# OATML-Markslab/ProteinGym

Hardware: AMD Instinct MI355X
Metric: mutants scored/sec (ESM-1v 650M masked-marginal) (higher is better)
Workload: dtype f16x3 (fp32 operands split into 2 fp16 planes, 3 fp16 MFMAs per product, fp32 accumulate)

## Files before the change

### proteingym_amd/csrc/api_esm.hip

```cpp
#include "model.h"

namespace pgmi {

int create_esm(pgmi_model* m, const pgmi_config* cfg, const float* w, int64_t n_weights) {
    BlobCursor c(m, w, n_weights);
    walk_esm(c);
    return c.finish();
}

void walk_esm_layer(BlobCursor& c, Layer* Lp, size_t F) {
    pgmi_model* m = c.m;
    const size_t D = m->cfg.embed_dim, dh = m->dh, Da = m->Da;
    auto slot = [&](size_t col) -> size_t { return rotate_half_slot(col, dh); };
    const float qscale = 1.0f / sqrtf((float)dh);
    std::vector<float> wq(3 * Da * D, 0.0f), bq(3 * Da, 0.0f), wo_r(D * Da, 0.0f);
    Layer& L = *Lp;
    c.upload(&L.ln1_w, D);
    c.upload(&L.ln1_b, D);
    pack_qkv_slots(c.take(3 * (D * D + D)), D, Da, slot, qscale, wq.data(), bq.data());
    c.linear(&L.wqkv, &L.wqkv16, wq.data(), wq.size(), D);
    c.upload(&L.bqkv, bq.data(), bq.size());
    pack_out_cols(c.take(D * D), D, Da, slot, wo_r.data());
    c.linear(&L.wo, &L.wo16, wo_r.data(), wo_r.size(), Da);
    c.upload(&L.bo, D);
    c.upload(&L.ln2_w, D);
    c.upload(&L.ln2_b, D);
    c.linear(&L.w1, &L.w116, F * D, D);
    c.upload(&L.b1, F);
    c.linear(&L.w2, &L.w216, D * F, F);
    c.upload(&L.b2, D);
}

void walk_esm(BlobCursor& c) {
    pgmi_model* m = c.m;
    const pgmi_config* cfg = &m->cfg;
    const size_t D = cfg->embed_dim, V = cfg->vocab;
    c.upload(&m->embed_tokens, V * D);
    if (cfg->arch == PGMI_ARCH_ESM1B) c.upload(&m->embed_positions, (size_t)(cfg->max_positions + 2) * D);
    if (cfg->emb_layer_norm_before) {
        c.upload(&m->lnb_w, D);
        c.upload(&m->lnb_b, D);
    }
    m->layers.resize(cfg->layers);
    for (int l = 0; l < cfg->layers; ++l) walk_esm_layer(c, &m->layers[l], cfg->ffn_dim);
    c.upload(&m->lna_w, D);
    c.upload(&m->lna_b, D);
    c.linear(&m->hd_w, &m->hd16, D * D, D);
    c.upload(&m->hd_b, D);
    c.upload(&m->hln_w, D);
    c.upload(&m->hln_b, D);
    c.upload(&m->head_b, V);
    m->head_w = m->embed_tokens;
}

int ensure_rotary(pgmi_model* m, int T) {
    if ((!esm2_rotary(m->cfg.arch) && !esmc_blocks(m->cfg.arch)) || T <= m->rot_len) return PGMI_OK;
    return upload_rotate_half(m, std::max(T, 1026));
}

int upload_rotate_half(pgmi_model* m, int n) {
    const int rh = m->rot_halves;
    float inv[64];
    const int half = m->dh / 2;
    for (int i = 0; i < half; ++i) inv[i] = 1.0f / powf(10000.0f, (float)(2 * i) / (float)m->dh);
    return upload_rotary(m, n, rh, [&](int t, int g, int i) {
        const int j = (rh == 1) ? i : 32 * g + i;
        return j < half ? (float)t * inv[j] : 0.0f;
    });
}

int encoder_layer(pgmi_model* m, const Layer& L, int B, int T, bool rotary, const int32_t* keep, int n_keep, bool* compacted) {
    const pgmi_config& c = m->cfg;
    const int M = B * T, D = c.embed_dim, F = L.ffn ? L.ffn : c.ffn_dim, N1 = L.ffn ? L.ffn : m->fc1_cols, H = c.heads, Da = m->Da;
    hipStream_t s = m->stream;
    int rc = PGMI_OK;
    const double ln_bytes = 2.0 * M * D * 4;
    const int prec = c.precision;
    const int mode16 = (prec == PGMI_PREC_F16X3) ? 1 : 2;
    { ProfScope p(m, PGMI_K_LAYERNORM, 0, ln_bytes);
      if (prec == PGMI_PREC_FP32) launch_layernorm(m->x, L.ln1_w, L.ln1_b, M, D, 1e-5f, m->h, s);
      else launch_layernorm16(m->x, L.ln1_w, L.ln1_b, M, D, 1e-5f, m->h16, mode16, s); }
    const bool fused_qkv = prec != PGMI_PREC_FP32 && !L.q_ln;
    { ProfScope p(m, PGMI_K_GEMM_QKV, 2.0 * M * 3 * D * D, 0);
      if (fused_qkv) {
          GemmLaunch g = qkv_launch(m, L.wqkv16, L.bqkv, M, Da, D, T, m->Hs);
          g.bf = prec == PGMI_PREC_BF16;
          g.qkv.cos_t = m->rot_cos; g.qkv.sin_t = m->rot_sin; g.qkv.rotary = rotary; g.qkv.rot_halves = m->rot_halves;
          rc = launch_gemm16(g);
      } else
          rc = linear(m, m->h, m->h16, L.wqkv, L.wqkv16, L.bqkv, nullptr, m->qkv, nullptr, M, 3 * Da, D, EPI_NONE);
      if (rc) return rc; }
    { ProfScope p(m, PGMI_K_ATTENTION, 4.0 * M * T * D, L.q_ln ? (double)M * D * 20 : 0);
      if (L.q_ln && (rc = launch_qkln_prep(m->qkv, L.q_ln, L.k_ln, 1e-5f, m->rot_cos, m->rot_sin, B, T, H, m->qk16, m->qk16_plane,
                                           m->vt16, m->vt16_plane, s)))
          return rc;
      const bool v2 = prec != PGMI_PREC_FP32;
      if (rotary && !v2) launch_rotary(m->qkv, m->rot_cos, m->rot_sin, M, T, m->Hs, s, m->rot_halves);
      if (v2) {
          AttLaunch a;
          a.qk16 = m->qk16, a.qk_plane = m->qk16_plane, a.vt16 = m->vt16, a.vt_plane = m->vt16_plane;
          a.B = B, a.T = T, a.H = H, a.head_dim = m->rot_halves * kHeadDim;
          a.kv_len = m->kv_len;
          a.out = prec == PGMI_PREC_F16X3 ? ATT_OUT_SPLIT : ATT_OUT_BF16;
          a.ctx16 = m->h16;
          a.stream = s;
          rc = launch_attention_f16x3_v2(a);
      } else {
          rc = launch_attention_f32(m->qkv, m->kv_len, B, T, H, m->h, s, m->rot_halves * kHeadDim);
      }
      if (rc) return rc; }
    if (keep && !L.g_norm_w) {
        const int R = n_keep;
        ProfScope p(m, PGMI_K_KEPT_ROWS, 2.0 * R * D * (Da + N1 + F), 0);
        launch_gather_rows(m->x, keep, R, D, m->qkv, s);
        if (prec == PGMI_PREC_FP32) launch_gather_rows(m->h, keep, R, Da, m->g, s);
        else
            launch_gather_rows(reinterpret_cast<const float*>(m->h16), keep, R, prec == PGMI_PREC_F16X3 ? Da : Da / 2,
                               reinterpret_cast<float*>(m->g16), s);
        rc = linear(m, m->g, m->g16, L.wo, L.wo16, L.bo, m->qkv, m->x, nullptr, R, D, Da, EPI_NONE);
        if (rc) return rc;
        if (prec == PGMI_PREC_FP32) launch_layernorm(m->x, L.ln2_w, L.ln2_b, R, D, 1e-5f, m->h, s);
        else launch_layernorm16(m->x, L.ln2_w, L.ln2_b, R, D, 1e-5f, m->h16, mode16, s);
        rc = linear(m, m->h, m->h16, L.w1, L.w116, L.b1, nullptr,
                    prec == PGMI_PREC_FP32 ? m->g : nullptr, prec == PGMI_PREC_FP32 ? nullptr : m->g16,
                    R, N1, D, m->fc1_epi);
        if (rc) return rc;
        rc = linear(m, m->g, m->g16, L.w2, L.w216, L.b2, m->x, m->x, nullptr, R, D, F, EPI_NONE);
        if (rc) return rc;
        if (compacted) *compacted = true;
        return PGMI_OK;
    }
    { ProfScope p(m, PGMI_K_GEMM_OUT, 2.0 * M * D * D, 0);
      rc = linear(m, m->h, m->h16, L.wo, L.wo16, L.bo, m->x, m->x, nullptr, M, D, Da, EPI_NONE);
      if (rc) return rc; }
    if (L.g_norm_w && m->e3_framed && (rc = geom_branch(m, L, B, T))) return rc;
    { ProfScope p(m, PGMI_K_LAYERNORM, 0, ln_bytes);
      if (prec == PGMI_PREC_FP32) launch_layernorm(m->x, L.ln2_w, L.ln2_b, M, D, 1e-5f, m->h, s);
      else launch_layernorm16(m->x, L.ln2_w, L.ln2_b, M, D, 1e-5f, m->h16, mode16, s); }
    { ProfScope p(m, PGMI_K_GEMM_FC1, 2.0 * M * N1 * D, 0);
      rc = linear(m, m->h, m->h16, L.w1, L.w116, L.b1, nullptr,
                  prec == PGMI_PREC_FP32 ? m->g : nullptr, prec == PGMI_PREC_FP32 ? nullptr : m->g16,
                  M, N1, D, m->fc1_epi);
      if (rc) return rc; }
    { ProfScope p(m, PGMI_K_GEMM_FC2, 2.0 * M * F * D, 0);
      rc = linear(m, m->g, m->g16, L.w2, L.w216, L.b2, m->x, m->x, nullptr, M, D, F, EPI_NONE);
      if (rc) return rc; }
    return PGMI_OK;
}

int run_encoder(pgmi_model* m, int B, int T, const int32_t* keep, int n_keep, bool* compacted) {
    const pgmi_config& c = m->cfg;
    const int M = B * T, D = c.embed_dim;
    hipStream_t s = m->stream;
    if (c.arch == PGMI_ARCH_ESM1B && T > c.max_positions) {
        set_error("Sequence length %d above maximum sequence length of %d", T, c.max_positions);
        return PGMI_EINVAL;
    }
    int rc = ensure_rotary(m, T);
    if (!rc) rc = reset_pad_keys(m, B, T);
    if (rc) return rc;
    {
        ProfScope p(m, PGMI_K_EMBED, 0, (double)M * D * 4);
        launch_seq_stats(m->tokens, B, T, m->embed_gather ? 0 : c.token_dropout, m->denom, m->pos_idx, m->kv_len, s, m->mask_id);
        if (c.arch == PGMI_ARCH_ESM3) { if ((rc = esm3_embed(m, B, T))) return rc; }
        else if (c.arch == PGMI_ARCH_MULAN) { if ((rc = mulan_embed(m, B, T))) return rc; }
        else if (m->embed_gather) launch_gather_rows(m->embed_tokens, m->tokens, M, D, m->x, s);
        else launch_embed(m->tokens, m->denom, m->pos_idx, m->embed_tokens, m->embed_positions, c.token_dropout, M, T, D, m->x, s, m->mask_id);
        if (m->lnb_w) {
            launch_layernorm(m->x, m->lnb_w, m->lnb_b, M, D, 1e-5f, m->x, s);
            launch_zero_pad_rows(m->tokens, M, D, m->x, s);
        }
    }
    for (int l = 0; l < c.layers; ++l) {
        const bool kept = keep && m->keep_rows && l == c.layers - 1;
        if ((rc = encoder_layer(m, m->layers[l], B, T, esm2_rotary(c.arch), kept ? keep : nullptr, n_keep, compacted))) return rc;
    }
    PGMI_HIP(hipGetLastError());
    return PGMI_OK;
}

int run_head(pgmi_model* m, int R, const int32_t* row_idx) {
    const pgmi_config& c = m->cfg;
    ProfScope p(m, PGMI_K_HEAD, 2.0 * R * c.embed_dim * (c.embed_dim + c.vocab), 0);
    int rc = head_hidden(m, R, row_idx);
    if (rc) return rc;
    launch_vocab_logsoftmax(m->g, m->head_w, m->head_b, R, c.embed_dim, c.vocab, m->lp, m->nonfinite, m->stream);
    PGMI_HIP(hipGetLastError());
    return PGMI_OK;
}

int head_hidden(pgmi_model* m, int R, const int32_t* row_idx) {
    const pgmi_config& c = m->cfg;
    const int D = c.embed_dim;
    hipStream_t s = m->stream;
    const int prec = c.precision;
    const float* src = m->x;
    if (row_idx) {
        launch_gather_rows(m->x, row_idx, R, D, m->h, s);
        src = m->h;
    }
    if (prec == PGMI_PREC_FP32) launch_layernorm(src, m->lna_w, m->lna_b, R, D, 1e-5f, m->h, s);
    else launch_layernorm16(src, m->lna_w, m->lna_b, R, D, 1e-5f, m->h16, prec == PGMI_PREC_F16X3 ? 1 : 2, s);
    int rc = linear(m, m->h, m->h16, m->hd_w, m->hd16, m->hd_b, nullptr, m->g, nullptr, R, D, D, EPI_GELU);
    if (rc) return rc;
    launch_layernorm(m->g, m->hln_w, m->hln_b, R, D, 1e-5f, m->g, s);
    return PGMI_OK;
}


int run_rows(pgmi_model* m, int B, int T, int R, const int32_t* row_idx) {
    bool compacted = false;
    int rc = run_encoder(m, B, T, row_idx, R, &compacted);
    if (rc) return rc;
    return run_head(m, R, compacted ? nullptr : row_idx);
}

}

extern "C" {

int pgmi_token_logprobs(pgmi_model* m, const int32_t* tokens, int B, int T, float* out) {
    if (!m || !tokens || !out || B <= 0 || T <= 0) { set_error("bad argument"); return PGMI_EINVAL; }
    if (m->cfg.arch == PGMI_ARCH_SAPROT) { set_error("SaProt models are scored with pgmi_saprot_token_logprobs / pgmi_saprot_group_logprobs"); return PGMI_EINVAL; }
    if (m->cfg.arch == PGMI_ARCH_MULAN) { set_error("MULAN models are scored with pgmi_mulan_token_logprobs / pgmi_mulan_set_logprobs"); return PGMI_EINVAL; }
    if (T + 31 > m->max_rows) { set_error("T=%d exceeds workspace rows %d", T, m->max_rows); return PGMI_EINVAL; }
    int rc = check_tokens(tokens, B, T);
    if (rc) return rc;
    PGMI_HIP(hipSetDevice(m->device));
    const int V = m->cfg.vocab;
    rc = for_each_chunk(m, B, T, [&](int b0, int bc) {
        PGMI_HIP(hipMemcpyAsync(m->tokens, tokens + (size_t)b0 * T, (size_t)bc * T * 4, hipMemcpyHostToDevice, m->stream));
        int rc = run_rows(m, bc, T, bc * T, nullptr);
        if (rc) return rc;
        PGMI_HIP(hipMemcpyAsync(out + (size_t)b0 * T * V, m->lp, (size_t)bc * T * V * 4, hipMemcpyDeviceToHost, m->stream));
        return PGMI_OK;
    });
    return rc ? rc : check_nonfinite(m);
}

int pgmi_masked_logprobs(pgmi_model* m, const int32_t* tokens, const int32_t* mask_pos, int B, int T, float* out) {
    if (!m || !tokens || !mask_pos || !out || B <= 0 || T <= 0) { set_error("bad argument"); return PGMI_EINVAL; }
    if (m->cfg.arch == PGMI_ARCH_SAPROT) { set_error("SaProt models are scored with pgmi_saprot_token_logprobs / pgmi_saprot_group_logprobs"); return PGMI_EINVAL; }
    if (m->cfg.arch == PGMI_ARCH_MULAN) { set_error("MULAN models are scored with pgmi_mulan_token_logprobs / pgmi_mulan_set_logprobs"); return PGMI_EINVAL; }
    if (esmc_blocks(m->cfg.arch) && T + 31 > m->max_rows) { set_error("T=%d exceeds workspace rows %d", T, m->max_rows); return PGMI_EINVAL; }
    if (T > m->max_rows) { set_error("T=%d exceeds workspace rows %d", T, m->max_rows); return PGMI_EINVAL; }
    int rc = check_tokens(tokens, B, T);
    if (rc) return rc;
    for (int b = 0; b < B; ++b)
        if (mask_pos[b] < 0 || mask_pos[b] >= T) { set_error("mask_pos[%d]=%d out of range", b, mask_pos[b]); return PGMI_EINVAL; }
    PGMI_HIP(hipSetDevice(m->device));
    const int V = m->cfg.vocab;
    std::vector<int32_t> ridx;
    rc = for_each_chunk(m, B, T, [&](int b0, int bc) {
        ridx.resize(bc);
        for (int b = 0; b < bc; ++b) ridx[b] = b * T + mask_pos[b0 + b];
        PGMI_HIP(hipMemcpyAsync(m->tokens, tokens + (size_t)b0 * T, (size_t)bc * T * 4, hipMemcpyHostToDevice, m->stream));
        PGMI_HIP(hipMemcpyAsync(m->aux_i, mask_pos + b0, (size_t)bc * 4, hipMemcpyHostToDevice, m->stream));
        PGMI_HIP(hipMemcpyAsync(m->row_idx, ridx.data(), (size_t)bc * 4, hipMemcpyHostToDevice, m->stream));
        launch_apply_mask(m->tokens, m->aux_i, bc, T, m->stream);
        int rc = run_rows(m, bc, T, bc, m->row_idx);
        if (rc) return rc;
        PGMI_HIP(hipMemcpyAsync(out + (size_t)b0 * V, m->lp, (size_t)bc * V * 4, hipMemcpyDeviceToHost, m->stream));
        return PGMI_OK;
    });
    return rc ? rc : check_nonfinite(m);
}

int pgmi_assay_create(pgmi_model* m, const int32_t* wt_tokens, int n_tok, const int32_t* positions, int P,
                      int window, const int32_t* sub_pos, const int32_t* sub_wt, const int32_t* sub_mt,
                      const int64_t* mut_off, int64_t n_mut, pgmi_assay** out) {
    if (!out) { set_error("null out"); return PGMI_EINVAL; }
    *out = nullptr;
    if (!m || !wt_tokens || n_tok <= 0 || P < 0 || (P > 0 && !positions) || window <= 0 || n_mut < 0) { set_error("bad argument"); return PGMI_EINVAL; }
    if (esmc_blocks(m->cfg.arch)) { set_error("ESM C / ESM3 assays run through pgmi_masked_logprobs (their window rule is not pgmi_optimal_window)"); return PGMI_EINVAL; }
    if (m->cfg.arch == PGMI_ARCH_SAPROT) { set_error("SaProt assays run through pgmi_saprot_group_logprobs (position sets, no window)"); return PGMI_EINVAL; }
    if (m->cfg.arch == PGMI_ARCH_MULAN) { set_error("MULAN assays run through pgmi_mulan_set_logprobs (position sets, no window)"); return PGMI_EINVAL; }
    for (int i = 0; i < n_tok; ++i)
        if (wt_tokens[i] < 0 || wt_tokens[i] >= PGMI_VOCAB || wt_tokens[i] == PGMI_TOK_PAD) { set_error("wt token %d invalid at %d", wt_tokens[i], i); return PGMI_EINVAL; }
    const int T = std::min(n_tok, window);
    if (T > m->max_rows) { set_error("T=%d exceeds workspace rows %d", T, m->max_rows); return PGMI_EINVAL; }
    std::vector<int32_t> ws(P), mr(P);
    for (int i = 0; i < P; ++i) {
        if (positions[i] < 0 || positions[i] >= n_tok) { set_error("position %d out of range", positions[i]); return PGMI_EINVAL; }
        int s, e;
        pgmi_optimal_window(positions[i], n_tok, window, &s, &e);
        if (e - s != T) { set_error("internal: window length %d != %d", e - s, T); return PGMI_EINVAL; }
        ws[i] = s;
        mr[i] = positions[i] - s;
    }
    const int64_t n_sub = n_mut ? mut_off[n_mut] : 0;
    for (int64_t k = 0; k < n_sub; ++k)
        if (sub_pos[k] < 0 || sub_pos[k] >= n_tok || sub_wt[k] < 0 || sub_wt[k] >= PGMI_VOCAB || sub_mt[k] < 0 || sub_mt[k] >= PGMI_VOCAB) {
            set_error("substitution %lld out of range", (long long)k);
            return PGMI_EINVAL;
        }
    PGMI_HIP(hipSetDevice(m->device));
    pgmi_assay* a = new pgmi_assay();
    a->m = m; a->n_tok = n_tok; a->P = P; a->T = T; a->n_mut = n_mut; a->n_sub = n_sub;
    int rc = dev_upload(a->allocs, &a->wt, wt_tokens, (size_t)n_tok);
    if (!rc) rc = dev_upload(a->allocs, &a->positions, positions, (size_t)P);
    if (!rc) rc = dev_upload(a->allocs, &a->win_start, ws.data(), (size_t)P);
    if (!rc) rc = dev_upload(a->allocs, &a->mask_rel, mr.data(), (size_t)P);
    if (!rc) rc = dev_upload(a->allocs, &a->sub_pos, sub_pos, (size_t)n_sub);
    if (!rc) rc = dev_upload(a->allocs, &a->sub_wt, sub_wt, (size_t)n_sub);
    if (!rc) rc = dev_upload(a->allocs, &a->sub_mt, sub_mt, (size_t)n_sub);
    if (!rc) rc = dev_upload(a->allocs, &a->mut_off, mut_off, (size_t)(n_mut + 1));
    if (!rc) rc = dev_alloc(a->allocs, &a->table, (size_t)n_tok * PGMI_VOCAB);
    if (!rc) rc = dev_alloc(a->allocs, &a->scores, (size_t)n_mut);
    if (rc) { pgmi_assay_destroy(a); return rc; }
    m->assays.push_back(a);
    *out = a;
    return PGMI_OK;
}

void pgmi_assay_destroy(pgmi_assay* a) {
    if (!a) return;
    if (a->m) {
        hipSetDevice(a->m->device);
        hipStreamSynchronize(a->m->stream);
        auto& v = a->m->assays;
        v.erase(std::remove(v.begin(), v.end(), a), v.end());
    }
    for (void* p : a->allocs) hipFree(p);
    delete a;
}

int pgmi_assay_run(pgmi_model* m, pgmi_assay* a, double* scores_host, float* table_host, double* scores_dev) {
    if (!m || !a || a->m != m) { set_error("bad model/assay handle (assay belongs to another or a destroyed model)"); return PGMI_EINVAL; }
    PGMI_HIP(hipSetDevice(m->device));
    hipStream_t s = m->stream;
    const int T = a->T, V = m->cfg.vocab;
    const int per = rows_per_chunk(m, T);
    launch_fill_f32(a->table, (int64_t)a->n_tok * V, NAN, s);
    for (int p0 = 0; p0 < a->P; p0 += per) {
        const int bc = std::min(per, a->P - p0);
        launch_make_masked_windows(a->wt, a->win_start + p0, a->mask_rel + p0, bc, T, m->tokens, s);
        launch_row_index(a->mask_rel + p0, bc, T, m->row_idx, s);
        int rc = run_rows(m, bc, T, bc, m->row_idx);
        if (rc) return rc;
        launch_scatter_rows(m->lp, a->positions + p0, bc, V, a->table, s);
    }
    {
        ProfScope p(m, PGMI_K_SCORE, 0, (double)a->n_sub * 20);
        launch_score_mutants(a->table, V, a->sub_pos, a->sub_wt, a->sub_mt, a->mut_off, a->n_mut, a->scores, s);
    }
    PGMI_HIP(hipGetLastError());
    if (scores_dev && a->n_mut) PGMI_HIP(hipMemcpyAsync(scores_dev, a->scores, (size_t)a->n_mut * 8, hipMemcpyDeviceToDevice, s));
    if (scores_host && a->n_mut) PGMI_HIP(hipMemcpyAsync(scores_host, a->scores, (size_t)a->n_mut * 8, hipMemcpyDeviceToHost, s));
    if (table_host) PGMI_HIP(hipMemcpyAsync(table_host, a->table, (size_t)a->n_tok * V * 4, hipMemcpyDeviceToHost, s));
    PGMI_HIP(hipStreamSynchronize(s));
    return check_nonfinite(m);
}

int pgmi_pppl_create(pgmi_model* m, const uint8_t* tokens, const int64_t* seq_off, int64_t n_seq, pgmi_pppl** out) {
    if (!out) { set_error("null out"); return PGMI_EINVAL; }
    *out = nullptr;
    if (!m || !tokens || !seq_off || n_seq <= 0 || n_seq > 0x7fffffff) { set_error("bad argument"); return PGMI_EINVAL; }
    if (m->cfg.arch != PGMI_ARCH_ESM1B && m->cfg.arch != PGMI_ARCH_ESM2) { set_error("pseudo-ppl needs an ESM-1b/1v/ESM2 model"); return PGMI_EINVAL; }
    if (seq_off[0] != 0) { set_error("seq_off[0] must be 0"); return PGMI_EINVAL; }
    for (int64_t n = 0; n < n_seq; ++n) {
        const int64_t len = seq_off[n + 1] - seq_off[n];
        if (len < 2 || len > (1 << 24)) { set_error("sequence %lld has %lld tokens", (long long)n, (long long)len); return PGMI_EINVAL; }
        const uint8_t* t = tokens + seq_off[n];
        for (int64_t i = 0; i < len; ++i)
            if (t[i] >= PGMI_VOCAB || t[i] == PGMI_TOK_PAD) { set_error("token id %d invalid at sequence %lld, position %lld", (int)t[i], (long long)n, (long long)i); return PGMI_EINVAL; }
    }
    PGMI_HIP(hipSetDevice(m->device));
    pgmi_pppl* q = new pgmi_pppl();
    q->m = m;
    q->N = n_seq;
    q->off.assign(seq_off, seq_off + n_seq + 1);
    int rc = dev_upload(q->allocs, &q->tok8, tokens, (size_t)seq_off[n_seq]);
    if (!rc) rc = dev_upload(q->allocs, &q->off_dev, seq_off, (size_t)n_seq + 1);
    if (rc) { for (void* p : q->allocs) hipFree(p); delete q; return rc; }
    m->pppls.push_back(q);
    *out = q;
    return PGMI_OK;
}

void pgmi_pppl_destroy(pgmi_pppl* q) {
    if (!q) return;
    if (q->m) {
        hipSetDevice(q->m->device);
        hipStreamSynchronize(q->m->stream);
        auto& v = q->m->pppls;
        v.erase(std::remove(v.begin(), v.end(), q), v.end());
    }
    for (void* p : q->allocs) hipFree(p);
    delete q;
}

int64_t pgmi_pppl_rows(const pgmi_pppl* q, int64_t first, int64_t count) {
    if (!q || first < 0 || count < 0 || first + count > q->N) return -1;
    int64_t r = 0;
    for (int64_t n = first; n < first + count; ++n) r += std::max<int64_t>(0, q->off[n + 1] - q->off[n] - 4);
    return r;
}

int pgmi_pppl_run(pgmi_model* m, pgmi_pppl* q, int64_t first, int64_t count, double* scores_host, float* terms_host,
                  double* scores_dev) {
    if (!m || !q || q->m != m) { set_error("bad model/library handle (library belongs to another or a destroyed model)"); return PGMI_EINVAL; }
    if (first < 0 || count <= 0 || first + count > q->N) { set_error("sequence range [%lld, %lld) outside the library of %lld", (long long)first, (long long)(first + count), (long long)q->N); return PGMI_EINVAL; }
    PGMI_HIP(hipSetDevice(m->device));
    hipStream_t s = m->stream;
    const int J = (int)count, V = m->cfg.vocab;
    std::vector<int32_t> sid(J);
    for (int j = 0; j < J; ++j) sid[j] = (int32_t)(first + j);
    auto len_of = [&](int32_t n) { return q->off[n + 1] - q->off[n]; };
    std::stable_sort(sid.begin(), sid.end(), [&](int32_t a, int32_t b) { return len_of(a) > len_of(b); });
    std::vector<int64_t> rp((size_t)J + 1);
    rp[0] = 0;
    for (int j = 0; j < J; ++j) rp[j + 1] = rp[j] + std::max<int64_t>(0, len_of(sid[j]) - 4);
    const int64_t R = rp[J];
    const int64_t Tmax = len_of(sid[0]);
    if (R > 0 && Tmax + 31 > m->max_rows) { set_error("T=%lld exceeds workspace rows %d", (long long)Tmax, m->max_rows); return PGMI_EINVAL; }
    if (R > 0 && m->cfg.arch == PGMI_ARCH_ESM1B && Tmax > m->cfg.max_positions) {
        set_error("Sequence length %lld above maximum sequence length of %d", (long long)Tmax, m->cfg.max_positions);
        return PGMI_EINVAL;
    }
    std::vector<void*> pool;
    auto cleanup = [&]() { for (void* p : pool) hipFree(p); };
    int32_t* d_sid = nullptr;
    int64_t* d_rp = nullptr;
    float* d_terms = nullptr;
    double* d_out = nullptr;
    int rc = dev_upload(pool, &d_sid, sid.data(), (size_t)J);
    if (!rc) rc = dev_upload(pool, &d_rp, rp.data(), (size_t)J + 1);
    if (!rc) rc = dev_alloc(pool, &d_terms, (size_t)R);
    if (!rc) rc = dev_alloc(pool, &d_out, (size_t)J);
    if (rc) { cleanup(); return rc; }
    q->last_rows = R; q->last_chunks = 0; q->last_tokens = 0; q->last_padded = 0;
    int j0 = 0;
    for (int64_t g0 = 0; g0 < R;) {
        while (rp[j0 + 1] <= g0) ++j0;
        const int T = (int)len_of(sid[j0]);
        const int bc = (int)std::min<int64_t>(rows_per_chunk(m, T), R - g0);
        launch_make_pppl_rows(q->tok8, q->off_dev, d_sid, d_rp, J, g0, bc, T, m->tokens, m->row_idx, m->aux_i, s);
        rc = run_rows(m, bc, T, bc, m->row_idx);
        if (rc) { hipStreamSynchronize(s); cleanup(); return rc; }
        launch_pppl_pick(m->lp, m->aux_i, bc, V, d_terms + g0, s);
        q->last_chunks += 1;
        q->last_padded += (int64_t)bc * T;
        g0 += bc;
        if ((q->last_chunks & 63) == 0 && g0 < R && (rc = check_nonfinite(m)) != PGMI_OK) { cleanup(); return rc; }
    }
    for (int j = 0; j < J; ++j) q->last_tokens += (rp[j + 1] - rp[j]) * len_of(sid[j]);
    {
        ProfScope p(m, PGMI_K_SCORE, 0, (double)R * 4);
        launch_pppl_sum(d_terms, d_rp, d_sid, J, first, d_out, s);
    }
    hipError_t e = hipGetLastError();
    if (e == hipSuccess && scores_dev) e = hipMemcpyAsync(scores_dev, d_out, (size_t)J * 8, hipMemcpyDeviceToDevice, s);
    if (e == hipSuccess && scores_host) e = hipMemcpyAsync(scores_host, d_out, (size_t)J * 8, hipMemcpyDeviceToHost, s);
    std::vector<float> sorted_terms;
    if (e == hipSuccess && terms_host && R > 0) {
        sorted_terms.resize((size_t)R);
        e = hipMemcpyAsync(sorted_terms.data(), d_terms, (size_t)R * 4, hipMemcpyDeviceToHost, s);
    }
    if (e == hipSuccess) e = hipStreamSynchronize(s);
    cleanup();
    if (e != hipSuccess) { set_error("pseudo-ppl run failed: %s", hipGetErrorString(e)); return PGMI_EHIP; }
    if (terms_host && R > 0) {
        std::vector<int64_t> dst((size_t)J + 1, 0);
        for (int k = 0; k < J; ++k) dst[k + 1] = dst[k] + std::max<int64_t>(0, len_of((int32_t)(first + k)) - 4);
        for (int j = 0; j < J; ++j)
            std::copy(sorted_terms.begin() + rp[j], sorted_terms.begin() + rp[j + 1], terms_host + dst[sid[j] - first]);
    }
    return check_nonfinite(m);
}

int pgmi_pppl_stats(const pgmi_pppl* q, int64_t* rows, int64_t* chunks, int64_t* tokens, int64_t* padded_tokens) {
    if (!q) { set_error("null library"); return PGMI_EINVAL; }
    if (rows) *rows = q->last_rows;
    if (chunks) *chunks = q->last_chunks;
    if (tokens) *tokens = q->last_tokens;
    if (padded_tokens) *padded_tokens = q->last_padded;
    return PGMI_OK;
}

}
```

### proteingym_amd/csrc/api_model.hip

```cpp
#include "model.h"

namespace pgmi {

static thread_local char g_err[1024] = "";
void set_error(const char* fmt, ...) {
    va_list ap;
    va_start(ap, fmt);
    vsnprintf(g_err, sizeof(g_err), fmt, ap);
    va_end(ap);
}

int prof_drain(pgmi_model* m) {
    if (m->events_used == 0) return PGMI_OK;
    PGMI_HIP(hipStreamSynchronize(m->stream));
    for (size_t i = 0; i < m->events_used; ++i) {
        float ms = 0.f;
        PGMI_HIP(hipEventElapsedTime(&ms, m->events[i].start, m->events[i].stop));
        m->prof_ms[m->events[i].cls] += ms;
    }
    m->events_used = 0;
    return PGMI_OK;
}

int check_cfg(const pgmi_config* c) {
// ... 240 lines not shown
    if (c->emb_layer_norm_before) n += 2 * D;
    n += (int64_t)c->layers * (2 * D + 4 * (D * D + D) + 2 * D + (F * D + F) + (D * F + D));
    n += 2 * D + (D * D + D) + 2 * D + V;
    return n;
}

int pgmi_model_create(const pgmi_config* cfg, const float* w, int64_t n_weights, int device, pgmi_model** out) {
    if (cfg && cfg->arch == PGMI_ARCH_PROGEN2) {
        if (out) *out = nullptr;
        set_error("ProGen2 models are created with pgmi_pg2_model_create (it takes rotary_dim)");
        return PGMI_EINVAL;
    }
    if (cfg && cfg->arch == PGMI_ARCH_GPT) {
        if (out) *out = nullptr;
        set_error("causal decoder models are created with pgmi_gpt_model_create (it takes pos_kind)");
        return PGMI_EINVAL;
    }
    if (cfg && cfg->arch == PGMI_ARCH_SAPROT) {
        if (out) *out = nullptr;
        set_error("SaProt models are created with pgmi_saprot_model_create (it takes the tokenizer's <mask> id)");
        return PGMI_EINVAL;
    }
    if (cfg && cfg->arch == PGMI_ARCH_MULAN) {
        if (out) *out = nullptr;
        set_error("MULAN models are created with pgmi_mulan_model_create (it takes the <mask> id and the vocabulary's groups)");
        return PGMI_EINVAL;
    }
    if (cfg && cfg->arch == PGMI_ARCH_POET) {
        if (out) *out = nullptr;
        set_error("PoET models are created with pgmi_poet_model_create (it takes final_norm)");
        return PGMI_EINVAL;
    }
    if (cfg && cfg->arch == PGMI_ARCH_PROGEN3) {
        if (out) *out = nullptr;
        set_error("ProGen3 models are created with pgmi_pg3_model_create (it takes pgmi_pg3_params)");
        return PGMI_EINVAL;
    }
    if (cfg && cfg->arch == PGMI_ARCH_ESM3) {
        if (out) *out = nullptr;
        set_error("ESM3 models are created with pgmi_esm3_model_create (it takes v_heads)");
        return PGMI_EINVAL;
    }
    if (cfg && cfg->arch == PGMI_ARCH_ESMIF1) {
        if (out) *out = nullptr;
        set_error("ESM-IF1 decoders are created with pgmi_esmif1_model_create (it takes the encoder width)");
        return PGMI_EINVAL;
    }
    return model_create(cfg, w, n_weights, device, out, 0);
}

}

namespace pgmi {

static int alloc_workspace(pgmi_model* m) {
    const pgmi_config& c = m->cfg;
    const size_t R = m->max_rows, D = c.embed_dim, V = c.vocab, Da = m->Da;
    const size_t F = c.arch == PGMI_ARCH_MULAN ? std::max<size_t>(c.ffn_dim, 4 * D) : c.ffn_dim;
    const size_t Dw = std::max(D, Da);
    const bool f32mode = c.precision == PGMI_PREC_FP32;
    int rc = PGMI_OK;
    auto alloc = [&](auto** p, size_t n) { if (!rc) rc = dev_alloc(m->allocs, p, n); };
    alloc(&m->x, R * D);
    alloc(&m->h, R * Dw);
    alloc(&m->qkv, R * 3 * Da);
    alloc(&m->g, R * (f32mode ? std::max(F, D) : D));
    if (!f32mode) {
        const size_t planes = c.precision == PGMI_PREC_F16X3 ? 2 : 1;
        m->h16_plane = R * Dw;
        m->g16_plane = R * F;
        alloc(&m->h16, m->h16_plane * planes);
        alloc(&m->g16, m->g16_plane * planes);
    }
    alloc(&m->nonfinite, (size_t)1);
    if (!f32mode) {
        m->qk16_plane = R * 2 * Da;
        m->vt16_plane = R * Da;
        alloc(&m->qk16, m->qk16_plane * 2);
        alloc(&m->vt16, m->vt16_plane * 2);
    }
    if (c.arch == PGMI_ARCH_MSA) {
        alloc(&m->xt, R * D);
        alloc(&m->msa_kv_len, (size_t)2048);
    }
    alloc(&m->lp, ((c.arch == PGMI_ARCH_GPT || c.arch == PGMI_ARCH_PROGEN3) && V > kWave ? (size_t)m->gpt_head_rows : R) * V);
    alloc(&m->denom, R);
    alloc(&m->tokens, R);
    alloc(&m->pos_idx, R);
    alloc(&m->kv_len, R);
    alloc(&m->row_idx, R);
    alloc(&m->aux_i, R);
    if (rc) return rc;
    PGMI_HIP(hipMemset(m->nonfinite, 0, 4));
    if (m->vt16) PGMI_HIP(hipMemset(m->vt16, 0, m->vt16_plane * 2 * sizeof(unsigned short)));
    return PGMI_OK;
}

int model_create(const pgmi_config* cfg, const float* w, int64_t n_weights, int device, pgmi_model** out, int arch_arg,
                 const pgmi_pg3_params* pg3) {
    if (!out) { set_error("null out"); return PGMI_EINVAL; }
    *out = nullptr;
    int rc = check_cfg(cfg);
    if (rc) return rc;
    if (cfg->arch == PGMI_ARCH_PROGEN3 && (rc = pg3_check(cfg, pg3))) return rc;
    if (cfg->arch == PGMI_ARCH_ESM3 && (rc = esm3_check(cfg, arch_arg))) return rc;
    if (cfg->arch == PGMI_ARCH_ESMIF1 && (rc = if1_check(cfg, arch_arg))) return rc;
    const int64_t need = cfg->arch == PGMI_ARCH_GPT ? gpt_weight_count(cfg, arch_arg)
                         : cfg->arch == PGMI_ARCH_PROGEN3 ? pg3_weight_count(cfg, pg3)
                         : cfg->arch == PGMI_ARCH_POET ? poet_weight_count(cfg, arch_arg)
                         : cfg->arch == PGMI_ARCH_ESM3 ? esm3_weight_count(cfg, arch_arg)
                         : cfg->arch == PGMI_ARCH_ESMIF1 ? if1_weight_count(cfg, arch_arg)
                         : cfg->arch == PGMI_ARCH_MULAN ? mulan_weight_count(cfg) : pgmi_weight_count(cfg);
    if (need < 0) { set_error("causal decoder pos_kind %d: must be PGMI_GPT_POS_ROTARY or PGMI_GPT_POS_LEARNED", arch_arg); return PGMI_EINVAL; }
    if (!w || n_weights != need) {
        set_error("weight blob has %lld elements, config needs %lld", (long long)n_weights, (long long)need);
        return PGMI_EINVAL;
    }
    const int ndev = pgmi_device_count();
    if (ndev <= 0) { set_error("no HIP device visible (libpgmi has no CPU fallback)"); return PGMI_ENODEV; }
    if (device < 0 || device >= ndev) { set_error("device %d out of range (%d visible)", device, ndev); return PGMI_EINVAL; }
    PGMI_HIP(hipSetDevice(device));
    pgmi_model* m = new pgmi_model();
    m->cfg = *cfg;
    m->device = device;
    if (hipStreamCreateWithFlags(&m->stream, hipStreamNonBlocking) != hipSuccess) { set_error("hipStreamCreate failed"); delete m; return PGMI_EHIP; }
    m->dh = cfg->embed_dim / cfg->heads;
    m->rot_halves = m->dh > 2 * kHeadDim ? 4 : m->dh > kHeadDim ? 2 : 1;
    m->Hs = cfg->heads * m->rot_halves;
    m->Da = m->Hs * kHeadDim;
    m->ln_eps = cfg->ln_eps > 0.f ? cfg->ln_eps : 1e-5f;
    m->max_rows = std::max(cfg->max_rows > 0 ? cfg->max_rows : 98304, 2048);
    const size_t V = cfg->vocab;
    const std::vector<float> zeros(std::max({3 * (size_t)m->Da, (V + 63) / 64 * 64, (size_t)cfg->embed_dim, V, (size_t)cfg->heads}), 0.0f);
    rc = dev_upload(m->allocs, &m->zeros, zeros.data(), zeros.size());
    m->fc1_cols = cfg->ffn_dim;
    if (!rc) switch (cfg->arch) {
        case PGMI_ARCH_TRANCEPTION: rc = create_tranception(m, cfg, w, n_weights); break;
        case PGMI_ARCH_MSA: rc = create_msa(m, cfg, w, n_weights); break;
        case PGMI_ARCH_PROGEN2: rc = create_progen2(m, cfg, w, n_weights, arch_arg); break;
        case PGMI_ARCH_GPT: rc = create_gpt(m, cfg, w, n_weights, arch_arg); break;
        case PGMI_ARCH_ESMC: rc = create_esmc(m, cfg, w, n_weights); break;
        case PGMI_ARCH_SAPROT: rc = create_saprot(m, cfg, w, n_weights, arch_arg); break;
        case PGMI_ARCH_MULAN: rc = create_mulan(m, cfg, w, n_weights, arch_arg); break;
        case PGMI_ARCH_POET: rc = create_poet(m, cfg, w, n_weights, arch_arg); break;
        case PGMI_ARCH_PROGEN3: rc = create_progen3(m, cfg, w, n_weights, pg3); break;
        case PGMI_ARCH_ESM3: rc = create_esm3(m, cfg, w, n_weights, arch_arg); break;
        case PGMI_ARCH_ESMIF1: rc = create_esmif1(m, cfg, w, n_weights, arch_arg); break;
        default: rc = create_esm(m, cfg, w, n_weights);
    }
    if (!rc) rc = alloc_workspace(m);
    if (rc) { pgmi_model_destroy(m); return rc; }
    m->keep_rows = env_int("PGMI_KEEP_ROWS", 1);
    gemm_options_from_env();
    m->gemm_variant = env_int("PGMI_GEMM_VARIANT", 0);
    *out = m;
    return PGMI_OK;
}

}

namespace pgmi {

int side_open(pgmi_model* pm, const char* name, const float* w, int64_t n_weights, int64_t want, bool scan_finite, int device, int precision,
              hipStream_t lend) {
    if (!w || n_weights != want) {
        set_error("%s weight blob has %lld elements, config needs %lld", name, (long long)n_weights, (long long)want);
        return PGMI_EINVAL;
    }
    for (int64_t i = 0; scan_finite && i < n_weights; ++i)
        if (!std::isfinite(w[i])) { set_error("%s: weight blob element %lld is not finite", name, (long long)i); return PGMI_EINVAL; }
    int n_dev = 0;
    if (hipGetDeviceCount(&n_dev) != hipSuccess || n_dev <= 0) { set_error("no HIP device (libpgmi has no CPU fallback)"); return PGMI_ENODEV; }
    if (device < 0 || device >= n_dev) { set_error("device %d out of range (%d visible)", device, n_dev); return PGMI_EINVAL; }
    PGMI_HIP(hipSetDevice(device));
    gemm_options_from_env();
    pm->device = device;
    pm->cfg.precision = precision;
    if (lend) pm->stream = lend;
    else if (hipStreamCreate(&pm->stream) != hipSuccess) { set_error("hipStreamCreate failed"); return PGMI_EHIP; }
    return PGMI_OK;
}

int side_sync(pgmi_model* pm, int rc, const char* what) {
    const hipError_t e1 = hipGetLastError(), e2 = hipStreamSynchronize(pm->stream);
    if (!rc && (e1 != hipSuccess || e2 != hipSuccess)) {
        set_error("%s failed: %s", what, hipGetErrorString(e1 != hipSuccess ? e1 : e2));
        rc = PGMI_EHIP;
    }
    return rc;
}

int overflow_error(int precision) {
    set_error("non-finite log-probabilities%s", precision == PGMI_PREC_F16X3
              ? ": an activation left the fp16 range in precision f16x3; re-run with precision fp32" : "");
    return PGMI_EOVERFLOW;
}

void side_release(pgmi_model* pm, bool own_stream) {
    hipSetDevice(pm->device);
    if (pm->stream) hipStreamSynchronize(pm->stream);
    for (ProfEvent& e : pm->events) { hipEventDestroy(e.start); hipEventDestroy(e.stop); }
    for (void* p : pm->allocs) hipFree(p);
    if (pm->stream && own_stream) hipStreamDestroy(pm->stream);
}

}

extern "C" {

void pgmi_model_destroy(pgmi_model* m) {
    if (!m) return;
    hipSetDevice(m->device);
    if (m->stream) hipStreamSynchronize(m->stream);
    for (pgmi_assay* a : m->assays) {
        for (void* p : a->allocs) hipFree(p);
        a->allocs.clear();
        a->m = nullptr;
    }
    m->assays.clear();
    for (pgmi_pppl* q : m->pppls) {
        for (void* p : q->allocs) hipFree(p);
        q->allocs.clear();
        q->m = nullptr;
    }
    m->pppls.clear();
    for (auto& e : m->events) { hipEventDestroy(e.start); hipEventDestroy(e.stop); }
    if (m->moe.counts_host) hipHostFree(m->moe.counts_host);
    for (void* p : m->allocs) hipFree(p);
    if (m->stream) hipStreamDestroy(m->stream);
    delete m;
}

int pgmi_model_device(const pgmi_model* m) { return m ? m->device : -1; }

int pgmi_set_option(const char* name, int64_t value) {
    if (!name) { set_error("null option name"); return PGMI_EINVAL; }
    int rc = gemm_set_option(name, (long long)value);
    if (rc) rc = att_set_option(name, (long long)value);
    if (rc) rc = eve_set_option(name, (long long)value);
    if (rc) rc = mpnn_set_option(name, (long long)value);
    if (rc) rc = unirep_set_option(name, (long long)value);
    if (rc) rc = s2f_set_option(name, (long long)value);
    if (rc) set_error("unknown option '%s' (gemm_half_tail, gemm_max_rows, att_xcd_local, att_v3, eve_max_rows, eve_fixed_sample, eve_prior_batch, mpnn_max_rows, unirep_max_rows, s2f_max_rows)", name);
    return rc;
}

int pgmi_synchronize(pgmi_model* m) {
    if (!m) { set_error("null model"); return PGMI_EINVAL; }
    PGMI_HIP(hipStreamSynchronize(m->stream));
    return PGMI_OK;
}

int pgmi_profile_enable(pgmi_model* m, int on) {
    if (!m) { set_error("null model"); return PGMI_EINVAL; }
    int rc = prof_drain(m);
    m->prof = on != 0;
    return rc;
}

int pgmi_profile_reset(pgmi_model* m) {
    if (!m) { set_error("null model"); return PGMI_EINVAL; }
    int rc = prof_drain(m);
    for (int i = 0; i < PGMI_K_COUNT; ++i) { m->prof_ms[i] = 0; m->prof_n[i] = 0; m->prof_flops[i] = 0; m->prof_bytes[i] = 0; }
    return rc;
}

int pgmi_profile_get(pgmi_model* m, int k, double* ms, int64_t* launches, double* flops, double* bytes) {
    if (!m || k < 0 || k >= PGMI_K_COUNT) { set_error("bad argument"); return PGMI_EINVAL; }
    int rc = prof_drain(m);
    if (rc) return rc;
    if (ms) *ms = m->prof_ms[k];
    if (launches) *launches = m->prof_n[k];
    if (flops) *flops = m->prof_flops[k];
    if (bytes) *bytes = m->prof_bytes[k];
    return PGMI_OK;
}

}
```

### proteingym_amd/csrc/attention_f16.hip

```cpp
#include <stdlib.h>
#include <string.h>
#include <algorithm>

#include "attention_f16_common.h"

namespace pgmi {

template <int WPB, int OUT, int NSTG, int DH = 64, bool RAG = false, int DO = DH>
__global__ __launch_bounds__(WPB * 64) void attention_f16x3_v2_kernel(
    const unsigned short* __restrict__ qk16, size_t qk_plane, const unsigned short* __restrict__ vt16,
    size_t vt_plane, const int32_t* __restrict__ kv_len, const float* __restrict__ slopes, int T, int H,
    int Tp, float* __restrict__ ctx, unsigned short* __restrict__ ctx16, RagMap rag, int dense_nblk, int nseq) {
    constexpr float defer_thr = kAttDefer;
    constexpr int NT = WPB * 64;
    constexpr int KCPR = DH / 8;
    constexpr int KCH = AKT * KCPR, VCH = DO * 4;
    constexpr int NSL = DH / DO;
    static_assert(NSL == 1 || (OUT == ATT_OUT_SPLIT && !RAG), "sliced context: split-plane output of dense launches only");
    constexpr int STG_CH = 2 * KCH + 2 * VCH;
    constexpr int NWI = STG_CH / 64;
    static_assert(NWI % WPB == 0, "the wave-instructions of a stage divide evenly over the waves");
    constexpr int NDMA = NWI / WPB;
    constexpr int NS = DH / 16, ND = DO / 32;
    extern __shared__ __attribute__((aligned(16))) u32x4 lds[];
// ... 108 lines not shown
            for (int s = 0; s < NS; ++s) {
                const int ci = r * KCPR + ((2 * s + kh) ^ k_swizzle<DH>(r));
                qh[s] = qbase[ci];
                ql[s] = qbase[KCH + ci];
            }
        }
        asm volatile("s_waitcnt lgkmcnt(0)" ::: "memory");
        __builtin_amdgcn_s_barrier();
        asm volatile("" ::: "memory");
#pragma unroll
        for (int t = 1; t < NSTG - 1; ++t)
            if (t < nkt) issue_tile(t, t);
    } else {
#pragma unroll
        for (int t = 0; t < NSTG - 1; ++t)
            if (t < nkt) issue_tile(t, t);
    }

    f32x16 om[ND], oc[ND];
#pragma unroll
    for (int dt = 0; dt < ND; ++dt)
#pragma unroll
        for (int v = 0; v < 16; ++v) { om[dt][v] = 0.f; oc[dt][v] = 0.f; }
    float m_run = -INFINITY, l_run = 0.f;
    constexpr float kInvLo = 1.0f / kLoScale;

    const f32x16 zero16 = {0.f, 0.f, 0.f, 0.f, 0.f, 0.f, 0.f, 0.f, 0.f, 0.f, 0.f, 0.f, 0.f, 0.f, 0.f, 0.f};
    auto wanted = [&](int kt) -> bool { return active && !(causal && kt * AKT > q0 + 31); };
    auto scores = [&](int buf, f32x16& sm, f32x16& sc) {
        const u32x4* Kb = lds + buf * STG_CH;
#pragma unroll
        for (int s = 0; s < NS; ++s) {
            const int ci = r * KCPR + ((2 * s + kh) ^ k_swizzle<DH>(r));
            const u32x4 kfh = Kb[ci], kfl = Kb[KCH + ci];
            sc = mfma_h(kfh, ql[s], s == 0 ? zero16 : sc);
            sc = mfma_h(kfl, qh[s], sc);
            sm = mfma_h(kfh, qh[s], s == 0 ? zero16 : sm);
        }
    };
    auto wait_tile = [&](int younger) {
        if (younger >= 2) asm volatile("s_waitcnt vmcnt(%0)" ::"n"(2 * NDMA) : "memory");
        else if (younger == 1) asm volatile("s_waitcnt vmcnt(%0)" ::"n"(NDMA) : "memory");
        else asm volatile("s_waitcnt vmcnt(0)" ::: "memory");
    };
    int cur = 0;
    for (int kt = 0; kt < nkt; ++kt) {
        wait_tile(min(NSTG - 2, nkt - 1 - kt));
        __builtin_amdgcn_s_barrier();
        asm volatile("" ::: "memory");
        if (kt + NSTG - 1 < nkt) issue_tile(kt + NSTG - 1, (cur == 0) ? NSTG - 1 : cur - 1);
        if (wanted(kt)) {
            const u32x4* Vb = lds + cur * STG_CH + 2 * KCH;
            f32x16 sm, sc;
            scores(cur, sm, sc);
            float st[16];
            if (causal) {
                const float kb = (float)(kt * AKT + 4 * kh);
#pragma unroll
                for (int v = 0; v < 16; ++v)
                    st[v] = fmaf(slope2, kb + (float)((v & 3) + 8 * (v >> 2)), fmaf(sc[v], kInvLo, sm[v]));
                if (kt * AKT + AKT - 1 > q0) {
#pragma unroll
                    for (int v = 0; v < 16; ++v) {
                        const int key = kt * AKT + (v & 3) + 8 * (v >> 2) + 4 * kh;
                        if (key > q0 + r) st[v] = -INFINITY;
                    }
                }
            } else {
#pragma unroll
                for (int v = 0; v < 16; ++v) st[v] = fmaf(sc[v], kInvLo, sm[v]);
            }
            if (kt * AKT + AKT > Tk) {
#pragma unroll
                for (int v = 0; v < 16; ++v) {
                    const int key = kt * AKT + (v & 3) + 8 * (v >> 2) + 4 * kh;
                    if (key >= Tk) st[v] = -INFINITY;
                }
            }
            float mloc = st[0];
#pragma unroll
            for (int v = 1; v < 16; ++v) mloc = fmaxf(mloc, st[v]);
            {
                const unsigned int mu = __builtin_bit_cast(unsigned int, mloc);
                const auto sw = __builtin_amdgcn_permlane32_swap(mu, mu, false, false);
                const unsigned int s0 = sw[0], s1 = sw[1];
                mloc = fmaxf(__builtin_bit_cast(float, s0), __builtin_bit_cast(float, s1));
            }
            const float m_new = fmaxf(m_run, mloc);
            if (!__all(m_new <= m_run + defer_thr)) {
                const bool moved = m_new > m_run + defer_thr;
                const float alpha = moved ? __builtin_amdgcn_exp2f(m_run - m_new) : 1.0f;
                l_run *= alpha;
#pragma unroll
                for (int dt = 0; dt < ND; ++dt)
#pragma unroll
                    for (int v = 0; v < 16; ++v) { om[dt][v] *= alpha; oc[dt][v] *= alpha; }
                if (moved) m_run = m_new;
            }
            const float mb = m_run - 10.0f;
            typedef float f32x2 __attribute__((ext_vector_type(2)));
#pragma unroll
            for (int v = 0; v < 16; v += 2) {
                const f32x2 dlt = f32x2{st[v], st[v + 1]} - f32x2{mb, mb};
                st[v] = __builtin_amdgcn_exp2f(dlt[0]);
                st[v + 1] = __builtin_amdgcn_exp2f(dlt[1]);
            }
            l_run += ((st[0] + st[1]) + (st[2] + st[3])) + ((st[4] + st[5]) + (st[6] + st[7])) +
                     (((st[8] + st[9]) + (st[10] + st[11])) + ((st[12] + st[13]) + (st[14] + st[15])));
#pragma unroll
            for (int m = 0; m < 2; ++m) {
                u32x4 ph, pl;
#pragma unroll
                for (int e = 0; e < 4; ++e) {
                    const u32x2 p = split_p(st[8 * m + 2 * e], st[8 * m + 2 * e + 1]);
                    ph[e] = p[0];
                    pl[e] = p[1];
                }
#pragma unroll
                for (int dt = 0; dt < ND; ++dt) {
                    const int ci = v_chunk(dt * 32 + r, m, kh);
                    const u32x4 vfh = Vb[ci], vfl = Vb[VCH + ci];
                    oc[dt] = mfma_h(vfh, pl, oc[dt]);
                    oc[dt] = mfma_h(vfl, ph, oc[dt]);
                    om[dt] = mfma_h(vfh, ph, om[dt]);
                }
            }
        }
        cur = (cur == NSTG - 1) ? 0 : cur + 1;
    }

    if (active) {
        const float l_tot = l_run + __shfl_xor(l_run, 32);
        const float inv = 1.0f / l_tot;
        const bool row_ok = q0 + r < T && q0 + r >= p0;
        const size_t orow = (size_t)(orow0 + max(min(q0 + r, T - 1), p0));
        if (OUT == ATT_OUT_BF16) store_ctx_bf16<ND>(om, oc, inv, kInvLo, row_ok, ctx16 + orow * (size_t)D + (size_t)h * DH, kh);
        else if (OUT == ATT_OUT_SPLIT) store_ctx_split<ND>(om, oc, inv, kInvLo, row_ok, ctx16 + orow * (size_t)(2 * D) + (size_t)((h * DH + d0) / 32) * 64, kh);
        else if (row_ok) store_ctx_f32<ND>(om, oc, inv, kInvLo, ctx + (size_t)(orow0 + q0 + r) * D + (size_t)h * DH + 4 * kh);
    }
}


using Att16v2Kernel = decltype(&attention_f16x3_v2_kernel<4, ATT_OUT_F32, 3, 64, false, 64>);
struct Att16v2Inst { int wpb, out, head_dim; bool rag; Att16v2Kernel fn; size_t lds_bytes; };
template <int WPB, int OUT, int NSTG, int DH, bool RAG = false, int DO = DH>
static constexpr Att16v2Inst att16v2_inst() {
    return {WPB, OUT, DH, RAG, attention_f16x3_v2_kernel<WPB, OUT, NSTG, DH, RAG, DO>, (size_t)NSTG * (8 * DH + 8 * DO) * 16};
}
static const Att16v2Inst kAtt16v2[] = {
    att16v2_inst<1, ATT_OUT_F32, 3, 64>(),   att16v2_inst<2, ATT_OUT_F32, 3, 64>(),   att16v2_inst<4, ATT_OUT_F32, 3, 64>(),
    att16v2_inst<1, ATT_OUT_SPLIT, 3, 64>(), att16v2_inst<2, ATT_OUT_SPLIT, 3, 64>(), att16v2_inst<4, ATT_OUT_SPLIT, 3, 64>(),
    att16v2_inst<1, ATT_OUT_BF16, 3, 64>(),  att16v2_inst<2, ATT_OUT_BF16, 3, 64>(),  att16v2_inst<4, ATT_OUT_BF16, 3, 64>(),
    att16v2_inst<1, ATT_OUT_SPLIT, 3, 64, true>(), att16v2_inst<2, ATT_OUT_SPLIT, 3, 64, true>(), att16v2_inst<4, ATT_OUT_SPLIT, 3, 64, true>(),
    att16v2_inst<4, ATT_OUT_F32, 3, 128>(),  att16v2_inst<4, ATT_OUT_SPLIT, 3, 128>(), att16v2_inst<4, ATT_OUT_BF16, 3, 128>(),
    att16v2_inst<4, ATT_OUT_SPLIT, 2, 256, false, 128>(),
};

static int launch_att16v2(const AttLaunch& a, int wpb, dim3 grid, const RagMap* rag, int dense_nblk) {
    for (const Att16v2Inst& k : kAtt16v2) {
        if (k.wpb != wpb || k.out != a.out || k.head_dim != a.head_dim || k.rag != (rag != nullptr)) continue;
        if (k.lds_bytes > 65536) {
            hipError_t e = hipFuncSetAttribute(reinterpret_cast<const void*>(k.fn), hipFuncAttributeMaxDynamicSharedMemorySize, (int)k.lds_bytes);
            if (e != hipSuccess) { set_error("hipFuncSetAttribute: %s", hipGetErrorString(e)); return PGMI_EHIP; }
        }
        hipLaunchKernelGGL(k.fn, grid, dim3(wpb * 64), k.lds_bytes, a.stream, a.qk16, a.qk_plane, a.vt16, a.vt_plane, a.kv_len, a.slopes,
                           a.T, a.H, (a.T + 31) / 32 * 32, a.ctx, a.ctx16, rag ? *rag : RagMap{}, dense_nblk, a.B);
        PGMI_HIP(hipGetLastError());
        return PGMI_OK;
    }
    set_error("attention_f16x3_v2: no kernel for %d waves, output %d, head_dim %d%s", wpb, (int)a.out, a.head_dim, rag ? ", ragged" : "");
    return PGMI_EINVAL;
}

static int g_att_xcd_local = -1;
int att_set_option(const char* name, long long value) {
    if (!strcmp(name, "att_xcd_local")) { g_att_xcd_local = (int)value; return PGMI_OK; }
    if (!strcmp(name, "att_v3")) { att_v3_set_option((int)value); return PGMI_OK; }
    return PGMI_EINVAL;
}
static dim3 dense_grid(int nblk, int H, int B, int* dense_nblk) {
    if (g_att_xcd_local == 0 || (g_att_xcd_local < 0 && nblk < 2)) { *dense_nblk = 0; return dim3(nblk, H, B); }
    *dense_nblk = nblk;
    const long long pairs = (long long)H * B, groups = (pairs + 7) / 8;
    return dim3((unsigned)(groups * 8 * nblk), 1, 1);
}

int att16_waves_per_block(int T) {
    const int n32 = (T + 31) / 32, nblk = (n32 + 3) / 4;
    const int wpb = (n32 + nblk - 1) / nblk;
    return wpb == 3 ? 4 : wpb;
}

static int check_operand_range(const char* who, const AttLaunch& a) {
    const unsigned long long Tp = (unsigned long long)(a.T + 31) / 32 * 32;
    const unsigned long long seq_bytes = (unsigned long long)a.T * 2ull * (unsigned long long)a.H * (unsigned long long)a.head_dim * 2ull;
    const unsigned long long vt_bytes = (unsigned long long)a.head_dim * Tp * 2ull;
    if ((unsigned long long)a.qk_plane * 2ull + seq_bytes >= (1ull << 32) || (unsigned long long)a.vt_plane * 2ull + vt_bytes >= (1ull << 32)) {
        set_error("%s: operand planes of %zu / %zu halfs exceed the 32-bit offset range of the K / V^T DMA "
                  "(plane stride + one sequence must stay below 4 GiB: create the model with a smaller max_rows)", who, a.qk_plane, a.vt_plane);
        return PGMI_EINVAL;
    }
    return PGMI_OK;
}

int launch_attention_f16x3_v2(const AttLaunch& a) {
    const int B = a.B, T = a.T, H = a.H, head_dim = a.head_dim;
    if (B <= 0 || T <= 0 || H <= 0 || a.out < ATT_OUT_F32 || a.out > ATT_OUT_BF16 || (head_dim != 64 && head_dim != 128 && head_dim != 256)) {
        set_error("attention_f16x3_v2: bad arguments B=%d T=%d H=%d out=%d head_dim=%d", B, T, H, (int)a.out, head_dim);
        return PGMI_EINVAL;
    }
    const int n32 = (T + 31) / 32, Tp = n32 * 32;
    int rc = check_operand_range("attention_f16x3_v2", a);
    if (rc) return rc;
    int dn = 0;
    if (head_dim == 256) {
        if (a.qkv || a.conv || !a.slopes || a.out != ATT_OUT_SPLIT) { set_error("attention_f16x3_v2: head_dim 256 is the causal, fused-QKV, split-plane-output flavour only"); return PGMI_EINVAL; }
        const dim3 grid = dense_grid((n32 + 3) / 4, 2 * H, B, &dn);
        return launch_att16v2(a, 4, grid, nullptr, dn);
    }
    if (head_dim == 128) {
        if (a.qkv || a.conv) { set_error("attention_f16x3_v2: head_dim 128 needs operands from the fused QKV projection"); return PGMI_EINVAL; }
        const dim3 grid = dense_grid((n32 + 3) / 4, H, B, &dn);
        return launch_att16v2(a, 4, grid, nullptr, dn);
    }
    if (a.qkv && a.conv && a.rotary) { set_error("attention_f16x3_v2: depth-wise convolution and rotary together are not a model this library knows"); return PGMI_EINVAL; }
    if (a.qkv && a.conv && H % 4) { set_error("attention_f16x3_v2: the depth-wise convolution has four head groups, H = %d is not a multiple of 4", H); return PGMI_EINVAL; }
    if (a.qkv && a.conv)
        launch_qkv_prep_conv(dim3(n32, H, B), a.stream, a.qkv, a.conv, T, H, Tp, a.qk16, a.qk_plane, a.vt16, a.vt_plane, nullptr);
    else if (a.qkv)
        launch_qkv_prep(dim3(n32, H, B), a.stream, a.qkv, a.cos_t, a.sin_t, a.rotary, T, H, Tp, a.qk16, a.qk_plane, a.vt16, a.vt_plane);
    const int wpb = att16_waves_per_block(T);
    const dim3 grid = dense_grid((n32 + wpb - 1) / wpb, H, B, &dn);
    return att_v3_serves(a) ? launch_att16v3(a, wpb, grid, dn) : launch_att16v2(a, wpb, grid, nullptr, dn);
}

int launch_attention_tr_ragged(const AttLaunch& a, const AttRagged& rg) {
    const int T = a.T, H = a.H;
    if (T <= 0 || H <= 0 || !a.qkv || !a.conv || !a.slopes || a.head_dim != 64 || a.out != ATT_OUT_SPLIT || rg.n_tiles <= 0 || rg.n_blocks <= 0) {
        set_error("attention_tr_ragged: bad arguments T=%d H=%d tiles=%d blocks=%d", T, H, rg.n_tiles, rg.n_blocks);
        return PGMI_EINVAL;
    }
    const int rc = check_operand_range("attention_tr_ragged", a);
    if (rc) return rc;
    const RagMap tiles{rg.seq_off, rg.seq_p, rg.seq_q, rg.seq_root, rg.seq_vt, rg.tile_seq, rg.tile_j};
    launch_qkv_prep_conv(dim3(rg.n_tiles, H, 1), a.stream, a.qkv, a.conv, T, H, (T + 31) / 32 * 32, a.qk16, a.qk_plane, a.vt16, a.vt_plane, &tiles);
    const RagMap rag{rg.seq_off, rg.seq_p, rg.seq_q, rg.seq_root, rg.seq_vt, rg.blk_seq, rg.blk_j};
    return launch_att16v2(a, att16_waves_per_block(T), dim3(rg.n_blocks, H, 1), &rag, 0);
}

}
```

### proteingym_amd/csrc/common.h

```cpp
#pragma once
#include <hip/hip_runtime.h>
#include <stdint.h>
#include <stddef.h>

#include "../../include/pgmi.h"

namespace pgmi {

void set_error(const char* fmt, ...);

#define PGMI_HIP(expr)                                                                   \
    do {                                                                                 \
        hipError_t _e = (expr);                                                          \
        if (_e != hipSuccess) {                                                          \
            pgmi::set_error("%s failed: %s (%s:%d)", #expr, hipGetErrorString(_e),       \
                            __FILE__, __LINE__);                                         \
            return PGMI_EHIP;                                                            \
        }                                                                                \
    } while (0)

typedef float f32x4 __attribute__((ext_vector_type(4)));
typedef float f32x16 __attribute__((ext_vector_type(16)));

constexpr int kWave = 64;
constexpr int kHeadDim = 64;

enum Epilogue { EPI_NONE = 0, EPI_GELU = 1, EPI_SQRELU = 2, EPI_GELU_TANH = 3,
                EPI_SWIGLU = 4,
                EPI_RELU = 5 };

constexpr float kLoScale = 2048.0f;
constexpr float kQLog2e = 1.4426950408889634f;

__host__ __device__ __forceinline__ size_t ki_off(size_t row, int k, int K) {
    return row * (size_t)(2 * K) + (size_t)(k >> 5) * 64 + (size_t)(k & 31);
}
#if defined(__HIPCC__)
__device__ __forceinline__ void split_act(float x, _Float16& hi, _Float16& lo) {
    hi = (fabsf(x) < 6.103515625e-05f) ? (_Float16)0.0f : (_Float16)x;
    lo = (_Float16)((x - (float)hi) * kLoScale);
}
typedef _Float16 f16x4 __attribute__((ext_vector_type(4)));
__device__ __forceinline__ void split_act4(f32x4 x, f16x4& hi, f16x4& lo) {
    f32x4 xz, lo32;
#pragma unroll
    for (int e = 0; e < 4; ++e) xz[e] = (fabsf(x[e]) < 6.103515625e-05f) ? 0.0f : x[e];
    hi = __builtin_convertvector(xz, f16x4);
    const f32x4 xs = x * f32x4{kLoScale, kLoScale, kLoScale, kLoScale};
#pragma unroll
    for (int e = 0; e < 4; ++e) lo32[e] = __builtin_fmaf((float)hi[e], -kLoScale, xs[e]);
    lo = __builtin_convertvector(lo32, f16x4);
}
__device__ __forceinline__ void split_act4_prod(f32x4 a, f32x4 b, f16x4& hi, f16x4& lo) {
    const f32x4 x = a * b;
    f32x4 xz, lo32;
#pragma unroll
    for (int e = 0; e < 4; ++e) xz[e] = (fabsf(x[e]) < 6.103515625e-05f) ? 0.0f : x[e];
    hi = __builtin_convertvector(xz, f16x4);
#pragma unroll
    for (int e = 0; e < 4; ++e) lo32[e] = __builtin_fmaf(a[e], b[e], -(float)hi[e]);
    lo = __builtin_convertvector(lo32 * f32x4{kLoScale, kLoScale, kLoScale, kLoScale}, f16x4);
}
__device__ __forceinline__ void store_split4(f32x4 o, unsigned short* y16, size_t row, int c, int lane, int D) {
    typedef _Float16 h4 __attribute__((ext_vector_type(4)));
    typedef unsigned int u32x2 __attribute__((ext_vector_type(2)));
    typedef unsigned int u32x4 __attribute__((ext_vector_type(4)));
    h4 hi, lo;
#pragma unroll
    for (int k = 0; k < 4; ++k) {
        _Float16 a, b;
        split_act(o[k], a, b);
        hi[k] = a;
        lo[k] = b;
    }
    const u32x2 H = __builtin_bit_cast(u32x2, hi), L = __builtin_bit_cast(u32x2, lo);
    const bool odd = lane & 1;
    const unsigned int s0 = odd ? H[0] : L[0], s1 = odd ? H[1] : L[1];
    const unsigned int r0 = __shfl_xor(s0, 1), r1 = __shfl_xor(s1, 1);
    const u32x4 out = odd ? u32x4{r0, r1, L[0], L[1]} : u32x4{H[0], H[1], r0, r1};
    *reinterpret_cast<u32x4*>(y16 + ki_off(row, 4 * (c & ~1), D) + (odd ? 32 : 0)) = out;
}
#endif

void launch_make_masked_windows(const int32_t* wt, const int32_t* win_start, const int32_t* mask_rel,
                                int B, int T, int32_t* tokens_out, hipStream_t s);
void launch_apply_mask(int32_t* tokens, const int32_t* mask_pos, int B, int T, hipStream_t s);
void launch_seq_stats(const int32_t* tokens, int B, int T, int token_dropout, float* scale,
                      int32_t* pos_idx, int32_t* kv_len, hipStream_t s, int mask_id = PGMI_TOK_MASK);
void launch_zero_pad_rows(const int32_t* tokens, int rows, int D, float* x, hipStream_t s);
void launch_embed(const int32_t* tokens, const float* scale, const int32_t* pos_idx,
                  const float* embed_tokens, const float* embed_positions, int token_dropout,
                  int rows, int T, int D, float* x, hipStream_t s, int mask_id = PGMI_TOK_MASK);
void launch_layernorm(const float* x, const float* w, const float* b, int rows, int D, float eps,
                      float* y, hipStream_t s);
void launch_gather_rows(const float* x, const int32_t* row_idx, int n, int D, float* y, hipStream_t s);
void launch_strided_index(int first, int stride, int n, int32_t* idx, hipStream_t s);
void launch_vocab_logsoftmax(const float* h, const float* E, const float* bias, int rows, int D,
                             int V, float* out, int32_t* nonfinite, hipStream_t s);
void launch_layernorm16(const float* x, const float* w, const float* b, int rows, int D, float eps,
                        unsigned short* y16, int mode, hipStream_t s);
int launch_rmsnorm16(const float* x, const float* w, int rows, int D, float eps, unsigned short* y16, hipStream_t s);
void launch_scatter_rows(const float* src, const int32_t* dst_row, int n, int V, float* table,
                         hipStream_t s);
void launch_row_index(const int32_t* mask_rel, int B, int T, int32_t* out, hipStream_t s);
void launch_fill_f32(float* p, int64_t n, float v, hipStream_t s);
void launch_seq_loglik(const float* lp, const int32_t* tokens, const int32_t* lens, int B, int T, int V,
                       const float* prior, const int32_t* a0, const int32_t* row0, const int32_t* n,
                       const int32_t* flip, float alpha, const float* eve, float beta, int eve_fallback, float* out, hipStream_t s);
void launch_seq_loglik_ragged(const float* lp, const int32_t* tokens, const int32_t* seq_off, const int32_t* seq_p,
                              const int32_t* seq_root, int B, int T, int V, const float* prior, const int32_t* a0,
                              const int32_t* row0, const int32_t* n, const int32_t* flip, float alpha, const float* eve, float beta,
                              int eve_fallback, float* out, hipStream_t s);
void launch_pg2_seq_loglik(const float* lp, const int32_t* col, const int32_t* n_kept, int B, int T, int V, float* out, hipStream_t s);
void launch_embed_learned(const int32_t* tokens, const float* E, const float* P, int rows, int T, int D, float* x, hipStream_t s);
void launch_embed_scaled_pos(const int32_t* tokens, const int32_t* pos, const float* E, const float* P, float scale, int rows, int D,
                             float* x, hipStream_t s);
void launch_wide_logsoftmax(const float* logits, int ldl, int rows, int V, const int32_t* tgt, float* out, int32_t* nonfinite,
                            hipStream_t s);
void launch_seq_sum(const float* terms, const int32_t* off, int B, double* out, hipStream_t s);
void launch_score_mutants(const float* table, int V, const int32_t* sub_pos, const int32_t* sub_wt,
                          const int32_t* sub_mt, const int64_t* mut_off, int64_t n_mut,
                          double* scores, hipStream_t s);
void launch_rotary(float* qkv, const float* cos_t, const float* sin_t, int rows, int T, int H,
                   hipStream_t s, int rot_halves = 1);
void launch_make_pppl_rows(const uint8_t* tok8, const int64_t* seq_off, const int32_t* sid, const int64_t* rp, int J,
                           int64_t g0, int bc, int T, int32_t* tokens, int32_t* row_idx, int32_t* target, hipStream_t s);
void launch_pppl_pick(const float* lp, const int32_t* target, int bc, int V, float* terms, hipStream_t s);
void launch_pppl_sum(const float* terms, const int64_t* rp, const int32_t* sid, int J, int64_t first, double* out, hipStream_t s);
void launch_saprot_rows(const int32_t* wt, const int32_t* set_off, const int32_t* set_pos, int s0, int bc, int T, int first, int groups,
                        int width, int32_t* tokens, int32_t* keep, hipStream_t s);
void launch_mulan_rows(const int32_t* wt, const int32_t* set_off, const int32_t* set_pos, int s0, int bc, int T, int mask_id,
                       const float* angles, const float* plddt, const float* W, const float* bias, int D, int32_t* tokens, int32_t* keep,
                       float* y, hipStream_t s);
void launch_mulan_embed(const int32_t* tokens, const float* scale, const float* E, const float* st, int token_dropout, int rows, int T,
                        int D, float* x, hipStream_t s, int mask_id);
int launch_group_logsoftmax(const float* h, const float* E, const float* bias, int rows, int D, int V, int first, int groups, int width,
                            float* full, float* group, int32_t* nonfinite, hipStream_t s);
int group_logsoftmax_check(int D, int V, int first, int groups, int width);

struct MoeRoute {
    const float* gate = nullptr;
    int E = 0, top_k = 0;
    const int32_t* tokens = nullptr;
    int pad_id = 0;
    int32_t* ids = nullptr;
    float* wts = nullptr;
};
int launch_rmsnorm_route(const float* x, const float* w, int rows, int D, float eps, unsigned short* y16, const MoeRoute& r, hipStream_t s);
int moe_perm_blocks(int n_entries);
void launch_moe_permute(const int32_t* ids, int n_entries, int E, int tile, int32_t* blk_cnt, int32_t* blk_base, int32_t* counts_seg,
                        int32_t* slot, hipStream_t s);
void launch_moe_gather(const unsigned short* h16, const int32_t* slot, int n_entries, int top_k, int D, unsigned short* a16, hipStream_t s);
void launch_moe_combine(const float* y, const int32_t* slot, const float* wts, int rows, int top_k, int D, float* x, hipStream_t s);
void launch_silu_split(const float* t, int rows, int F, unsigned short* g16, hipStream_t s);

enum EveTensor { PGMI_EVE_T_Z = 0, PGMI_EVE_T_KEEP = 1, PGMI_EVE_T_W = 16, PGMI_EVE_T_B = 32, PGMI_EVE_T_WOUT = 48, PGMI_EVE_T_BOUT = 49,
                 PGMI_EVE_T_CONV = 50, PGMI_EVE_T_SPARSITY = 51, PGMI_EVE_T_TEMP = 52 };
void launch_eve_gather(const uint8_t* res, const float* W0t, const float* b, int rows, int L, int ld, int act, float* out, hipStream_t s);
void launch_eve_act(float* x, int rows, int n, int ld, int act, uint32_t keep24, float scale, uint64_t seed, uint32_t sample, int tensor,
                    int64_t row_base, const uint8_t* inj, int64_t inj_row0, hipStream_t s);
void launch_eve_latent(const float* mulv, int ldz, int64_t mulv_row0, int rows, int z, int ld, uint32_t keep24, float scale, uint64_t seed,
                       uint32_t sample, int64_t row_base, const float* inj_eps, const uint8_t* inj_keep, int64_t inj_row0, float* h,
                       hipStream_t s);
void launch_eve_sample(const float* mean, const float* sd, int64_t n, int K, int Kp, uint64_t seed, uint32_t sample, int tensor,
                       const float* inj, float* out, hipStream_t s);
void launch_eve_sample_final(const float* w_mean, const float* w_sd, const float* c_mean, const float* c_sd, const float* s_mean,
                             const float* s_sd, int L, int H, int Hp, int C, int Ht, bool conv, uint64_t seed, uint32_t sample,
                             const float* inj_w, const float* inj_c, const float* inj_s, float* out, hipStream_t s);
void launch_eve_elbo(const float* logits, const uint8_t* res, const float* mulv, int ldz, int z, const float* temp, int rows, int L,
                     int64_t loc0, float* elbo, float* bce, float* kld, double* acc, int first, hipStream_t s);
void launch_eve_fill_normal(uint64_t seed, uint32_t sample, int tensor, uint64_t e0, int64_t n, float* out, hipStream_t s);
void launch_eve_fill_keep(uint64_t seed, uint32_t sample, int tensor, uint64_t e0, int64_t n, uint32_t keep24, uint8_t* out, hipStream_t s);
constexpr int EVE_PRIOR_S = 4;
struct EvePriorPtrs { const float* p[EVE_PRIOR_S] = {nullptr, nullptr, nullptr, nullptr}; };
void launch_eve_prior_latent(const float* mulv, int z, int ld, uint64_t seed, uint32_t sample, const EvePriorPtrs& inj, int S, float* h,
                             hipStream_t s);
void launch_eve_prior_hidden(const float* w_mean, const float* w_sd, const float* b_mean, const float* b_sd, int N, int K, uint64_t seed,
                             uint32_t sample, int tw, int tb, const EvePriorPtrs& inj_w, const EvePriorPtrs& inj_b, int S, const float* x,
                             int ldx, int act, float* y, int ldy, hipStream_t s);
int eve_prior_blocks(int L, int H);
int eve_prior_kmax(int H);
int eve_prior_max_samples(int C, bool conv);
void launch_eve_prior_final(const float* w_mean, const float* w_sd, const float* c_mean, const float* c_sd, const float* s_mean,
                            const float* s_sd, int L, int H, int C, int Ht, bool conv, uint64_t seed, uint32_t sample,
                            const EvePriorPtrs& inj_w, const EvePriorPtrs& inj_c, const EvePriorPtrs& inj_s, int S, const float* h, int ldh,
                            float* partial, hipStream_t s);
void launch_eve_prior_finish(const float* partial, int S, const float* b_mean, const float* b_sd, const float* t_mean, const float* t_sd,
                             uint64_t seed, uint32_t sample, const EvePriorPtrs& inj_b, const EvePriorPtrs& inj_t, int L, int H, int sample0,
                             double* acc, hipStream_t s);
int eve_set_option(const char* name, long long value);

void launch_mpnn_graph(const float* X, const float* mask, int L, int K, int32_t* E_idx, float* D_nb, hipStream_t s);
void launch_mpnn_edge_feat(const float* X, const int32_t* ridx, const int32_t* chain, const int32_t* E_idx, const float* D_nb,
                           const float* Wpos, const float* bpos, const float* Wt, const float* ln_w, const float* ln_b, int L, int K, float* E,
                           hipStream_t s);
void launch_mpnn_concat(const float* hV, const float* hE, const int32_t* E_idx, int L, int K, float* out, hipStream_t s);
void launch_mpnn_edge_sum(const float* msg, const float* mask, const int32_t* E_idx, int L, int K, float* out, hipStream_t s);
void launch_mpnn_add_ln(const float* a, int64_t a_rows, const float* b, const float* bias, float kb, float div, const float* ln_w,
                        const float* ln_b, const float* rowmask, int L, int64_t rows, float* out, hipStream_t s);
int launch_mpnn_dec_edge(const float* Ep, const float* T, const float* Penc, const float* AP, int64_t ap_bstride, const float* W2,
                         const float* b2, const int32_t* E_idx, const float* mask, const uint8_t* S, const int32_t* rank, int B, int L, int K,
                         float* out, hipStream_t s);
void launch_mpnn_head(const float* h, const float* W, const float* bias, const uint8_t* S, int64_t rows, float* lp, float* nll,
                      hipStream_t s);
void launch_mpnn_score(const float* nll, const float* mask, int B, int L, double* out, hipStream_t s);
int mpnn_set_option(const char* name, long long value);

constexpr int S2F_S = 256, S2F_V = 16, S2F_H0 = 33;
struct S2fMsgWeights {
    const float *wv0, *wsv0, *bsv0;
    const float *wh1, *ws1, *bs1, *wv1, *wsv1, *bsv1;
    const float *wh2, *ws2, *bs2, *wv2, *wsv2, *bsv2;
    int ldw;
};
int launch_s2f_message(const float* P, const float* VT, const float* Es, const float* ev, const float* whe, const float* Wnt,
                       const S2fMsgWeights& w, const int32_t* src, const int32_t* off, int L, int64_t nodes, float* ds, float* dv, hipStream_t s);
int launch_s2f_gvp_mid(const float* spre, const float* vh, const float* wv, const float* gpre, const float* nwh, int so,
                       int vo, int h, int h2, int relu, int lda, int64_t rows, float* outA, float* outV, hipStream_t s);
int launch_s2f_node_ln(const float* rs, const float* rv, const float* ds, const float* dv, const float* lnw, const float* lnb, const float* wh, int h, int vn, int lda, int64_t rows, float* os, float* ov,
                       float* outA, float* outV, hipStream_t s);
void launch_s2f_head(const float* x, const float* sums, const int32_t* grp, int Ns, const float* W, const float* bias, const float* seq,
                     const float* plddt, float thr, int L, int64_t rows, float* lp, hipStream_t s);
void launch_s2f_pick_logits(const float* lp, const int32_t* cols, int L, int T, int V, int64_t rows, float* out, hipStream_t s);
int s2f_set_option(const char* name, long long value);

constexpr int S3F_DEG = 16;
int launch_s3f_knn(const float* q, int nq, const float* c, int nc, int k, int32_t* idx, float* dist, hipStream_t s);
void launch_s3f_edges(const float* pos, const int32_t* src, int Ns, const float* we, float* es, float* ev, hipStream_t s);
int launch_s3f_rows(const float* Z, const float* T, const int32_t* res, const float* lnw, const float* lnb, int L, int Ns, int H, int64_t rows,
                    float* out, hipStream_t s);
int launch_s3f_message(const float* P, const float* VT, const float* Es, const float* ev, const float* whe, const float* Wnt,
                       const S2fMsgWeights& w, const int32_t* src, int Ns, int64_t nodes, float* ds, float* dv, hipStream_t s);
int s3f_colsum_blocks(int Ns);
void launch_s3f_colsum(const float* x, int Ns, int copies, float* part, float* sums, hipStream_t s);

void launch_egnn_edge_rows(const float* P, const float* S, const int32_t* centre, const int32_t* nb, int edges, int Hp, bool split, void* out,
                           hipStream_t s);
void launch_egnn_aggregate(const float* x, const float* msg, const int32_t* off, const int32_t* eid, int L, int D, int hp, bool split, void* out,
                           hipStream_t s);
void launch_egnn_silu_rows(const float* t, int rows, int F, float* out, hipStream_t s);
void launch_egnn_head(const float* x, const float* W, const float* bias, int rows, int D, float* lp, hipStream_t s);

void launch_packed_scatter(const float* src, const int32_t* dst_row, int n, int D, float* out, int32_t* nonfinite, hipStream_t s);
void launch_vespag_head(const float* h, const float* W2, const float* b2, const int32_t* wt_col, int rows, int H, float slope, float* y,
                        hipStream_t s);

void launch_mlstm_m(const float* g1, const float* Tmx, const int32_t* tok, int tok_stride, int rows, int Hp, unsigned short* m16,
                    float* m32, hipStream_t s);
// ... 21 lines not shown
                          int n_seg, int64_t M, int C, int taps, int dilation, float* out32, hipStream_t s);
int launch_dilated_conv32(const float* x, const float* W, const float* bias, const int32_t* seg_off, int n_seg, int64_t M, int C, int taps,
                          int dilation, float* col, float* out32, hipStream_t s);
int launch_ln_gelu16(const float* x, const float* w, const float* b, int rows, int D, float eps, unsigned short* y16, hipStream_t s);
int launch_ln_gelu32(const float* x, const float* w, const float* b, int rows, int D, float eps, float* y, hipStream_t s);

void launch_msa_window_tokens(const int32_t* full, int R, int Tfull, int start, int Tw, int mask_col, int32_t* out, hipStream_t s);
void launch_add_row_embedding(float* x, const float* pe, int R, int C, int D, hipStream_t s);
void launch_permute_rows(const float* src, float* dst, int A, int B, int D, hipStream_t s);
void launch_tied_prep_qk(const float* qkv, int64_t M, int D, unsigned short* q16, unsigned short* k16, hipStream_t s);
void launch_pack_vt16(const float* qkv, int R, int C, int Kp, int H, unsigned short* Vt, hipStream_t s);
int launch_tied_softmax16(const float* part, int H, int S, int C, int Kp, float scale, unsigned short* P, hipStream_t s);
float tied_w_scale();
struct TiedRowLaunch {
    const float* qkv = nullptr;
    int R = 0, C = 0, H = 0;
    int S = 0;
    unsigned short* qctx16 = nullptr;
    unsigned short* k16 = nullptr;
    float* part = nullptr;
    float* p = nullptr;
    float* vt = nullptr;
    hipStream_t stream = nullptr;
};
int tied_row_kp(int C);
int tied_row_splits(int R, int C, int H);
int tied_row_check(int R, int C, int H, int S);
int launch_tied_row_attention(const TiedRowLaunch& t);

int launch_gemm_f32(const float* A, const float* W, const float* bias, const float* residual,
                    float* C, int M, int N, int K, int epilogue, hipStream_t s);

void gemm_options_from_env();
int gemm_set_option(const char* name, long long value);
struct GemmLaunch {
    const unsigned short* A = nullptr;
    const unsigned short* W = nullptr;
    float out_scale = 1.0f;
    const float* bias = nullptr;
    const float* residual = nullptr;
    float* out32 = nullptr;
    unsigned short* out16 = nullptr;
    int M = 0, N = 0, K = 0;
    int epilogue = EPI_NONE;
    bool bf = false;
    int variant = 0;
    hipStream_t stream = nullptr;
    struct Qkv {
        unsigned short* vt16 = nullptr;
        size_t vt_plane = 0, qk_plane = 0;
        const float* cos_t = nullptr;
        const float* sin_t = nullptr;
        int rotary = 0, T = 0, H = 0, rot_halves = 1;
    } qkv;
};
int launch_gemm16(const GemmLaunch& g);
struct XMap;
int launch_gemm16_ex(const unsigned short* A, const unsigned short* W, float* Cf, unsigned short* Ch, int M, int N, int K,
                     float out_scale, XMap xm, int nbatch, hipStream_t s);
void launch_split16(const float* x, int64_t n, float scale, int mode, int K, unsigned short* out, hipStream_t s);

int launch_qkln_prep(const float* qkv, const float* q_w, const float* k_w, float eps, const float* cos_t, const float* sin_t, int B,
                     int T, int H, unsigned short* qk16, size_t qk_plane, unsigned short* vt16, size_t vt_plane, hipStream_t s);

struct GeomAttLaunch {
    const float* proj = nullptr;
    int pitch = 0;
    const float *rot = nullptr, *trans = nullptr;
    const int32_t* mask = nullptr;
    bool per_row_frames = false;
    const float *w_rot = nullptr, *w_dist = nullptr;
    int B = 0, S = 0, H = 0;
    float* out = nullptr;
    int opitch = 0;
    hipStream_t stream = nullptr;
};
int launch_geom_attention(const GeomAttLaunch& g);
int geom_key_tile(int S);
void launch_esm3_embed(const int32_t* tokens, const int32_t* stok, const int32_t* plddt, const float* seq_embed, const float* struct_embed,
                       const float* cst, int rows, int T, int D, float* x, hipStream_t s);

int launch_attention_f32(const float* qkv, const int32_t* kv_len, int B, int T, int H, float* ctx, hipStream_t s,
                         int head_dim = 64);

enum AttOut {
    ATT_OUT_F32 = 0,
    ATT_OUT_SPLIT = 1,
    ATT_OUT_BF16 = 2
};
struct AttLaunch {
    unsigned short* qk16 = nullptr;
    size_t qk_plane = 0;
    unsigned short* vt16 = nullptr;
    size_t vt_plane = 0;
    int B = 1, T = 0, H = 0;
    int head_dim = 64;
    const int32_t* kv_len = nullptr;
    const float* slopes = nullptr;
    AttOut out = ATT_OUT_F32;
    float* ctx = nullptr;
    unsigned short* ctx16 = nullptr;
    hipStream_t stream = nullptr;
    const float* qkv = nullptr;
    const float* conv = nullptr;
    const float* cos_t = nullptr;
    const float* sin_t = nullptr;
    int rotary = 0;
};
int launch_attention_f16x3_v2(const AttLaunch& a);

struct AttRagged {
    const int32_t* seq_off;
    const int32_t* seq_p;
    const int32_t* seq_q;
    const int32_t* seq_root;
    const uint32_t* seq_vt;
    const int32_t* tile_seq;
    const int32_t* tile_j;
    const int32_t* blk_seq;
    const int32_t* blk_j;
    int n_tiles, n_blocks;
};
struct PrefixAttLaunch {
    const float* qkv = nullptr;
    const int32_t* pos = nullptr;
    const float* cos_t = nullptr;
    const float* sin_t = nullptr;
    const int32_t* seg_off = nullptr;
    const int32_t* ent_seg = nullptr;
    const int32_t* ent_tile = nullptr;
    int n_seg = 0, n_ent = 0, H = 0;
    unsigned short* q16 = nullptr;
    size_t q_plane = 0;
    unsigned short* k16 = nullptr;
    unsigned short* vt16 = nullptr;
    size_t pitch = 0;
    const unsigned short* pk16 = nullptr;
    const unsigned short* pvt16 = nullptr;
    size_t ppitch = 0;
    int P = 0;
    AttOut out = ATT_OUT_SPLIT;
    float* ctx = nullptr;
    unsigned short* ctx16 = nullptr;
    hipStream_t stream = nullptr;
};
int launch_prefix_prep(const PrefixAttLaunch& p);
int launch_prefix_attention(const PrefixAttLaunch& p);
int launch_cross_q_prep(const float* q, size_t rows, int H, unsigned short* q16, size_t q_plane, hipStream_t s);
int launch_cross_attention(const PrefixAttLaunch& p);

int att16_waves_per_block(int T);
int att_set_option(const char* name, long long value);
int launch_attention_tr_ragged(const AttLaunch& a, const AttRagged& rg);

}
```

### proteingym_amd/csrc/elementwise.hip

```cpp
#include "common.h"

namespace pgmi {

__device__ __forceinline__ float wave_sum(float v) {
#pragma unroll
    for (int o = 32; o > 0; o >>= 1) v += __shfl_xor(v, o);
    return v;
}
__device__ __forceinline__ float wave_max(float v) {
#pragma unroll
    for (int o = 32; o > 0; o >>= 1) v = fmaxf(v, __shfl_xor(v, o));
    return v;
}
__device__ __forceinline__ double wave_sum_d(double v) {
#pragma unroll
    for (int o = 32; o > 0; o >>= 1) v += __shfl_xor(v, o);
    return v;
}
__device__ __forceinline__ int wave_sum_i(int v) {
#pragma unroll
    for (int o = 32; o > 0; o >>= 1) v += __shfl_xor(v, o);
    return v;
}

// ... 131 lines not shown
            }
        }
    }
    const float rstd = 1.0f / sqrtf(wave_sum(q) / (float)D + eps);
    const f32x4* wr = reinterpret_cast<const f32x4*>(w);
    const f32x4* br = reinterpret_cast<const f32x4*>(bsh);
#pragma unroll
    for (int i = 0; i < NV; ++i) {
        const int c = lane + 64 * i;
        if (c < nv) {
            const f32x4 wv = wr[c], bv = br[c];
            f32x4 o;
#pragma unroll
            for (int k = 0; k < 4; ++k) o[k] = (v[i][k] - mean) * rstd * wv[k] + bv[k];
            if constexpr (OUTMODE == 0) {
                reinterpret_cast<f32x4*>(y + (size_t)row * D)[c] = o;
            } else if constexpr (OUTMODE == 1) {
                typedef _Float16 h4 __attribute__((ext_vector_type(4)));
                h4 hi, lo;
#pragma unroll
                for (int k = 0; k < 4; ++k) {
                    _Float16 a, b2;
                    split_act(o[k], a, b2);
                    hi[k] = a;
                    lo[k] = b2;
                }
                typedef unsigned int u32x2 __attribute__((ext_vector_type(2)));
                typedef unsigned int u32x4 __attribute__((ext_vector_type(4)));
                const u32x2 H = __builtin_bit_cast(u32x2, hi), L = __builtin_bit_cast(u32x2, lo);
                const bool odd = lane & 1;
                const unsigned int s0 = odd ? H[0] : L[0], s1 = odd ? H[1] : L[1];
                const unsigned int r0 = __shfl_xor(s0, 1), r1 = __shfl_xor(s1, 1);
                const u32x4 out = odd ? u32x4{r0, r1, L[0], L[1]} : u32x4{H[0], H[1], r0, r1};
                unsigned short* dst = y16 + ki_off((size_t)row, 4 * (c & ~1), D) + (odd ? 32 : 0);
                *reinterpret_cast<u32x4*>(dst) = out;
            } else {
                typedef unsigned int u32x2 __attribute__((ext_vector_type(2)));
                unsigned short b[4];
#pragma unroll
                for (int k = 0; k < 4; ++k) {
                    const float ok = o[k];
                    unsigned int u = __builtin_bit_cast(unsigned int, ok);
                    u += 0x7fffu + ((u >> 16) & 1u);
                    b[k] = (unsigned short)(u >> 16);
                }
                u32x2 pk;
                pk[0] = b[0] | ((unsigned)b[1] << 16);
                pk[1] = b[2] | ((unsigned)b[3] << 16);
                reinterpret_cast<u32x2*>(y16 + (size_t)row * D)[c] = pk;
            }
        }
    }
}
template <int OUTMODE>
static void launch_ln_mode(const float* x, const float* w, const float* b, int rows, int D, float eps,
                           float* y, unsigned short* y16, hipStream_t s) {
    const dim3 grid((rows + 3) / 4), block(256);
    const int nv = (D / 4 + 63) / 64;
    if (nv <= 1) hipLaunchKernelGGL((layernorm_kernel<1, OUTMODE>), grid, block, 0, s, x, w, b, rows, D, eps, y, y16);
    else if (nv <= 2) hipLaunchKernelGGL((layernorm_kernel<2, OUTMODE>), grid, block, 0, s, x, w, b, rows, D, eps, y, y16);
    else if (nv <= 5) hipLaunchKernelGGL((layernorm_kernel<5, OUTMODE>), grid, block, 0, s, x, w, b, rows, D, eps, y, y16);
    else if (nv <= 10) hipLaunchKernelGGL((layernorm_kernel<10, OUTMODE>), grid, block, 0, s, x, w, b, rows, D, eps, y, y16);
    else hipLaunchKernelGGL((layernorm_kernel<20, OUTMODE>), grid, block, 0, s, x, w, b, rows, D, eps, y, y16);
}
void launch_layernorm(const float* x, const float* w, const float* b, int rows, int D, float eps,
                      float* y, hipStream_t s) {
    launch_ln_mode<0>(x, w, b, rows, D, eps, y, nullptr, s);
}
void launch_layernorm16(const float* x, const float* w, const float* b, int rows, int D, float eps,
                        unsigned short* y16, int mode, hipStream_t s) {
    if (mode == 1) launch_ln_mode<1>(x, w, b, rows, D, eps, nullptr, y16, s);
    else launch_ln_mode<2>(x, w, b, rows, D, eps, nullptr, y16, s);
}

template <int NV>
__global__ __launch_bounds__(256) void rmsnorm16_kernel(const float* __restrict__ x, const float* __restrict__ w, int rows, int D,
                                                        float eps, unsigned short* __restrict__ y16) {
    const int row = blockIdx.x * 4 + (threadIdx.x >> 6);
    const int lane = threadIdx.x & 63;
    if (row >= rows) return;
    const int nv = D >> 2;
    const f32x4* xr = reinterpret_cast<const f32x4*>(x + (size_t)row * D);
    f32x4 v[NV];
    float q = 0.f;
#pragma unroll
    for (int i = 0; i < NV; ++i) {
        const int c = lane + 64 * i;
        v[i] = (c < nv) ? xr[c] : f32x4{0.f, 0.f, 0.f, 0.f};
        q += (v[i][0] * v[i][0] + v[i][1] * v[i][1]) + (v[i][2] * v[i][2] + v[i][3] * v[i][3]);
    }
    const float rstd = 1.0f / sqrtf(wave_sum(q) / (float)D + eps);
    const f32x4* wr = reinterpret_cast<const f32x4*>(w);
#pragma unroll
    for (int i = 0; i < NV; ++i) {
        const int c = lane + 64 * i;
        if (c < nv) {
            const f32x4 wv = wr[c];
            f32x4 o;
#pragma unroll
            for (int k = 0; k < 4; ++k) o[k] = v[i][k] * rstd * wv[k];
            store_split4(o, y16, (size_t)row, c, lane, D);
        }
    }
}
int launch_rmsnorm16(const float* x, const float* w, int rows, int D, float eps, unsigned short* y16, hipStream_t s) {
    if (rows <= 0 || D <= 0 || D % 32 || D > 5120) { set_error("rmsnorm: D = %d must be a multiple of 32, at most 5120", D); return PGMI_EINVAL; }
    const dim3 grid((rows + 3) / 4), block(256);
    const int nv = (D / 4 + 63) / 64;
    if (nv <= 1) hipLaunchKernelGGL((rmsnorm16_kernel<1>), grid, block, 0, s, x, w, rows, D, eps, y16);
    else if (nv <= 2) hipLaunchKernelGGL((rmsnorm16_kernel<2>), grid, block, 0, s, x, w, rows, D, eps, y16);
    else if (nv <= 5) hipLaunchKernelGGL((rmsnorm16_kernel<5>), grid, block, 0, s, x, w, rows, D, eps, y16);
    else if (nv <= 10) hipLaunchKernelGGL((rmsnorm16_kernel<10>), grid, block, 0, s, x, w, rows, D, eps, y16);
    else hipLaunchKernelGGL((rmsnorm16_kernel<20>), grid, block, 0, s, x, w, rows, D, eps, y16);
    return PGMI_OK;
}

__global__ void rotary_kernel(float* __restrict__ qkv, const float* __restrict__ cos_t,
                              const float* __restrict__ sin_t, int64_t n, int T, int H, int rh) {
    const int64_t i = (int64_t)blockIdx.x * blockDim.x + threadIdx.x;
    if (i >= n) return;
    const int d = (int)(i & 31);
    const int64_t j = i >> 5;
    const int h = (int)(j % H);
    const int64_t k2 = j / H;
    const int which = (int)(k2 & 1);
    const int64_t row = k2 >> 1;
    const int t = (int)(row % T);
    float* p = qkv + row * (size_t)(3 * H * 64) + (size_t)which * H * 64 + h * 64 + d;
    const float x1 = p[0], x2 = p[32];
    const int tr = (t * rh + (h % rh)) * 64;
    const float c1 = cos_t[tr + d], s1 = sin_t[tr + d];
    const float c2 = cos_t[tr + d + 32], s2 = sin_t[tr + d + 32];
    p[0] = x1 * c1 + (-x2) * s1;
    p[32] = x2 * c2 + x1 * s2;
}
void launch_rotary(float* qkv, const float* cos_t, const float* sin_t, int rows, int T, int H, hipStream_t s, int rot_halves) {
    const int64_t n = (int64_t)rows * 2 * H * 32;
    hipLaunchKernelGGL(rotary_kernel, dim3((unsigned)((n + 255) / 256)), dim3(256), 0, s, qkv, cos_t, sin_t, n, T, H, rot_halves);
}

__global__ void gather_rows_kernel(const float* __restrict__ x, const int32_t* __restrict__ idx, int n,
                                   int D, float* __restrict__ y) {
    const int row = blockIdx.x * 4 + (threadIdx.x >> 6);
    const int lane = threadIdx.x & 63;
    if (row >= n) return;
    const f32x4* src = reinterpret_cast<const f32x4*>(x + (size_t)idx[row] * D);
    f32x4* dst = reinterpret_cast<f32x4*>(y + (size_t)row * D);
    for (int i = lane; i < D / 4; i += 64) dst[i] = src[i];
}
void launch_gather_rows(const float* x, const int32_t* idx, int n, int D, float* y, hipStream_t s) {
    hipLaunchKernelGGL(gather_rows_kernel, dim3((n + 3) / 4), dim3(256), 0, s, x, idx, n, D, y);
}

__global__ void esm3_embed_kernel(const int32_t* __restrict__ tokens, const int32_t* __restrict__ stok, const int32_t* __restrict__ plddt,
                                  const float* __restrict__ seq_embed, const float* __restrict__ struct_embed, const float* __restrict__ cst,
                                  int n, int T, int D, float* __restrict__ x) {
    const int row = blockIdx.x * 4 + (threadIdx.x >> 6);
    const int lane = threadIdx.x & 63;
    if (row >= n) return;
    const int t = row % T;
    const f32x4* a = reinterpret_cast<const f32x4*>(seq_embed + (size_t)tokens[row] * D);
    const f32x4* b = reinterpret_cast<const f32x4*>(struct_embed + (size_t)stok[t] * D);
    const f32x4* c = reinterpret_cast<const f32x4*>(cst + (size_t)(plddt[t] != 0) * D);
    f32x4* dst = reinterpret_cast<f32x4*>(x + (size_t)row * D);
    for (int i = lane; i < D / 4; i += 64) dst[i] = (a[i] + b[i]) + c[i];
}
void launch_esm3_embed(const int32_t* tokens, const int32_t* stok, const int32_t* plddt, const float* seq_embed, const float* struct_embed,
                       const float* cst, int rows, int T, int D, float* x, hipStream_t s) {
    hipLaunchKernelGGL(esm3_embed_kernel, dim3((rows + 3) / 4), dim3(256), 0, s, tokens, stok, plddt, seq_embed, struct_embed, cst, rows, T, D, x);
}

__global__ void strided_index_kernel(int first, int stride, int n, int32_t* __restrict__ idx) {
    const int i = blockIdx.x * blockDim.x + threadIdx.x;
    if (i < n) idx[i] = first + i * stride;
}
void launch_strided_index(int first, int stride, int n, int32_t* idx, hipStream_t s) {
    hipLaunchKernelGGL(strided_index_kernel, dim3((n + 255) / 256), dim3(256), 0, s, first, stride, n, idx);
}

__global__ void scatter_rows_kernel(const float* __restrict__ src, const int32_t* __restrict__ dst_row,
                                    int n, int V, float* __restrict__ table) {
    const int i = blockIdx.x * blockDim.x + threadIdx.x;
    if (i >= n * V) return;
    const int rI = i / V, c = i % V;
    table[(size_t)dst_row[rI] * V + c] = src[i];
}
void launch_scatter_rows(const float* src, const int32_t* dst_row, int n, int V, float* table, hipStream_t s) {
    hipLaunchKernelGGL(scatter_rows_kernel, dim3((n * V + 255) / 256), dim3(256), 0, s, src, dst_row, n, V, table);
}

__global__ void row_index_kernel(const int32_t* __restrict__ mask_rel, int B, int T, int32_t* __restrict__ out) {
    const int b = blockIdx.x * blockDim.x + threadIdx.x;
    if (b < B) out[b] = b * T + mask_rel[b];
}
void launch_row_index(const int32_t* mask_rel, int B, int T, int32_t* out, hipStream_t s) {
    hipLaunchKernelGGL(row_index_kernel, dim3((B + 255) / 256), dim3(256), 0, s, mask_rel, B, T, out);
}

__global__ void fill_f32_kernel(float* p, int64_t n, float v) {
    const int64_t i = (int64_t)blockIdx.x * blockDim.x + threadIdx.x;
    if (i < n) p[i] = v;
}
void launch_fill_f32(float* p, int64_t n, float v, hipStream_t s) {
    hipLaunchKernelGGL(fill_f32_kernel, dim3((unsigned)((n + 255) / 256)), dim3(256), 0, s, p, n, v);
}

__global__ __launch_bounds__(256) void vocab_logsoftmax_kernel(const float* __restrict__ h,
                                                               const float* __restrict__ E,
                                                               const float* __restrict__ bias, int rows,
                                                               int D, int V, float* __restrict__ out,
                                                               int32_t* __restrict__ nonfinite) {
    const int row = blockIdx.x * 4 + (threadIdx.x >> 6);
    const int lane = threadIdx.x & 63;
    if (row >= rows) return;
    const float* hr = h + (size_t)row * D;
    double my_logit = -INFINITY;
    for (int v = 0; v < V; ++v) {
        const float* ev = E + (size_t)v * D;
        double acc = 0.0;
        for (int i = lane; i < D; i += 64) acc = fma((double)hr[i], (double)ev[i], acc);
        acc = wave_sum_d(acc);
        if (lane == v) my_logit = acc + (double)bias[v];
    }
    const float mx = wave_max((float)my_logit);
    const double ex = (lane < V) ? exp(my_logit - (double)mx) : 0.0;
    const double lse = log(wave_sum_d(ex));
    const float res = (float)((my_logit - (double)mx) - lse);
    if (lane < V) {
        out[(size_t)row * V + lane] = res;
        if (nonfinite && !(fabsf(res) <= 3.0e38f)) atomicOr(nonfinite, 1);
    }
}
void launch_vocab_logsoftmax(const float* h, const float* E, const float* bias, int rows, int D, int V,
                             float* out, int32_t* nonfinite, hipStream_t s) {
    hipLaunchKernelGGL(vocab_logsoftmax_kernel, dim3((rows + 3) / 4), dim3(256), 0, s, h, E, bias, rows, D, V, out, nonfinite);
}

__device__ __forceinline__ float fuse_eve(float two, float e, float beta, int eve_fallback) {
    if (eve_fallback && e == -INFINITY) return two;
    return (1.0f - beta) * two + beta * e;
}
__global__ __launch_bounds__(256) void seq_loglik_kernel(const float* __restrict__ lp, const int32_t* __restrict__ tokens,
                                                         const int32_t* __restrict__ lens, int B, int T, int V,
                                                         const float* __restrict__ prior, const int32_t* __restrict__ a0,
                                                         const int32_t* __restrict__ row0, const int32_t* __restrict__ n,
                                                         const int32_t* __restrict__ flip, float alpha,
                                                         const float* __restrict__ eve, float beta, int eve_fallback,
                                                         float* __restrict__ out) {
    const int b = blockIdx.x * 4 + (threadIdx.x >> 6);
    const int lane = threadIdx.x & 63;
    if (b >= B) return;
    const int len = lens[b];
    float acc = 0.f;
    for (int t = lane; t < len - 1; t += 64) {
        const int tgt = tokens[(size_t)b * T + t + 1];
        float v = lp[((size_t)b * T + t) * V + tgt];
        if (prior && n[b] > 0 && t >= a0[b] && t < a0[b] + n[b]) {
            const int i = t - a0[b];
            const int row = flip[b] ? row0[b] + (n[b] - 1 - i) : row0[b] + i;
            v = (1.0f - alpha) * v + alpha * prior[(size_t)row * V + tgt];
            if (eve) v = fuse_eve(v, eve[(size_t)row * V + tgt], beta, eve_fallback);
        }
        acc += v;
    }
    acc = wave_sum(acc);
    if (lane == 0) out[b] = acc;
}
__global__ __launch_bounds__(256) void seq_loglik_ragged_kernel(const float* __restrict__ lp, const int32_t* __restrict__ tokens,
                                                                const int32_t* __restrict__ seq_off, const int32_t* __restrict__ seq_p,
                                                                const int32_t* __restrict__ seq_root, int B, int T, int V,
                                                                const float* __restrict__ prior, const int32_t* __restrict__ a0,
                                                                const int32_t* __restrict__ row0, const int32_t* __restrict__ n,
                                                                const int32_t* __restrict__ flip, float alpha,
                                                                const float* __restrict__ eve, float beta, int eve_fallback,
                                                                float* __restrict__ out) {
    const int b = blockIdx.x * 4 + (threadIdx.x >> 6);
    const int lane = threadIdx.x & 63;
    if (b >= B) return;
    const int a = seq_p[b], own0 = seq_off[b] - a, root0 = seq_off[seq_root[b]];
    float acc = 0.f;
    for (int t = lane; t < T - 1; t += 64) {
        const int tgt = tokens[(t + 1 < a) ? root0 + t + 1 : own0 + t + 1];
        float v = lp[(size_t)((t < a) ? root0 + t : own0 + t) * V + tgt];
        if (prior && n[b] > 0 && t >= a0[b] && t < a0[b] + n[b]) {
            const int i = t - a0[b];
            const int row = flip[b] ? row0[b] + (n[b] - 1 - i) : row0[b] + i;
            v = (1.0f - alpha) * v + alpha * prior[(size_t)row * V + tgt];
            if (eve) v = fuse_eve(v, eve[(size_t)row * V + tgt], beta, eve_fallback);
        }
        acc += v;
    }
    acc = wave_sum(acc);
    if (lane == 0) out[b] = acc;
}
void launch_seq_loglik_ragged(const float* lp, const int32_t* tokens, const int32_t* seq_off, const int32_t* seq_p,
                              const int32_t* seq_root, int B, int T, int V, const float* prior, const int32_t* a0,
                              const int32_t* row0, const int32_t* n, const int32_t* flip, float alpha, const float* eve, float beta,
                              int eve_fallback, float* out, hipStream_t s) {
    hipLaunchKernelGGL(seq_loglik_ragged_kernel, dim3((B + 3) / 4), dim3(256), 0, s, lp, tokens, seq_off, seq_p, seq_root, B, T, V,
                       prior, a0, row0, n, flip, alpha, eve, beta, eve_fallback, out);
}
void launch_seq_loglik(const float* lp, const int32_t* tokens, const int32_t* lens, int B, int T, int V,
                       const float* prior, const int32_t* a0, const int32_t* row0, const int32_t* n,
                       const int32_t* flip, float alpha, const float* eve, float beta, int eve_fallback, float* out, hipStream_t s) {
    hipLaunchKernelGGL(seq_loglik_kernel, dim3((B + 3) / 4), dim3(256), 0, s, lp, tokens, lens, B, T, V, prior, a0, row0, n,
                       flip, alpha, eve, beta, eve_fallback, out);
}

__global__ __launch_bounds__(256) void pg2_seq_loglik_kernel(const float* __restrict__ lp, const int32_t* __restrict__ col,
                                                             const int32_t* __restrict__ n_kept, int B, int T, int V,
                                                             float* __restrict__ out) {
    const int b = blockIdx.x * 4 + (threadIdx.x >> 6);
    const int lane = threadIdx.x & 63;
    if (b >= B) return;
    const int n = n_kept[b];
    double acc = 0.0;
    for (int t = lane; t < n; t += 64) acc += (double)lp[((size_t)b * T + t) * V + col[(size_t)b * T + t]];
    acc = wave_sum_d(acc);
    if (lane == 0) out[b] = (float)acc;
}
void launch_pg2_seq_loglik(const float* lp, const int32_t* col, const int32_t* n_kept, int B, int T, int V, float* out, hipStream_t s) {
    hipLaunchKernelGGL(pg2_seq_loglik_kernel, dim3((B + 3) / 4), dim3(256), 0, s, lp, col, n_kept, B, T, V, out);
}

__global__ void score_mutants_kernel(const float* __restrict__ table, int V,
                                     const int32_t* __restrict__ sub_pos,
                                     const int32_t* __restrict__ sub_wt,
                                     const int32_t* __restrict__ sub_mt,
                                     const int64_t* __restrict__ mut_off, int64_t n_mut,
                                     double* __restrict__ scores) {
    const int64_t i = (int64_t)blockIdx.x * blockDim.x + threadIdx.x;
    if (i >= n_mut) return;
    double sc = 0.0;
    for (int64_t k = mut_off[i]; k < mut_off[i + 1]; ++k) {
        const float* rowp = table + (size_t)sub_pos[k] * V;
        const float d = rowp[sub_mt[k]] - rowp[sub_wt[k]];
        sc += (double)d;
    }
    scores[i] = sc;
}
void launch_score_mutants(const float* table, int V, const int32_t* sub_pos, const int32_t* sub_wt,
                          const int32_t* sub_mt, const int64_t* mut_off, int64_t n_mut, double* scores,
                          hipStream_t s) {
    if (n_mut <= 0) return;
    hipLaunchKernelGGL(score_mutants_kernel, dim3((unsigned)((n_mut + 255) / 256)), dim3(256), 0, s, table, V,
                       sub_pos, sub_wt, sub_mt, mut_off, n_mut, scores);
}


__global__ __launch_bounds__(256) void make_pppl_rows_kernel(const uint8_t* __restrict__ tok8, const int64_t* __restrict__ seq_off,
                                                             const int32_t* __restrict__ sid, const int64_t* __restrict__ rp, int J,
                                                             int64_t g0, int bc, int T, int32_t* __restrict__ tokens,
                                                             int32_t* __restrict__ row_idx, int32_t* __restrict__ target) {
    const int b = blockIdx.x * 4 + (threadIdx.x >> 6);
    const int lane = threadIdx.x & 63;
    if (b >= bc) return;
    const int64_t g = g0 + b;
    int lo = 0, hi = J;
    while (hi - lo > 1) {
        const int mid = (lo + hi) >> 1;
        if (rp[mid] <= g) lo = mid; else hi = mid;
    }
    const int n = sid[lo];
    const int i = 1 + (int)(g - rp[lo]);
    const int64_t o = seq_off[n];
    const int len = (int)(seq_off[n + 1] - o);
    int32_t* out = tokens + (int64_t)b * T;
    for (int t = lane; t < T; t += 64) out[t] = (t == i) ? PGMI_TOK_MASK : (t < len ? (int32_t)tok8[o + t] : PGMI_TOK_PAD);
    if (lane == 0) {
        row_idx[b] = b * T + i;
        target[b] = (int32_t)tok8[o + i + 1];
    }
}
void launch_make_pppl_rows(const uint8_t* tok8, const int64_t* seq_off, const int32_t* sid, const int64_t* rp, int J,
                           int64_t g0, int bc, int T, int32_t* tokens, int32_t* row_idx, int32_t* target, hipStream_t s) {
    hipLaunchKernelGGL(make_pppl_rows_kernel, dim3((bc + 3) / 4), dim3(256), 0, s, tok8, seq_off, sid, rp, J, g0, bc, T,
                       tokens, row_idx, target);
}

__global__ void pppl_pick_kernel(const float* __restrict__ lp, const int32_t* __restrict__ target, int bc, int V,
                                 float* __restrict__ terms) {
    const int b = blockIdx.x * blockDim.x + threadIdx.x;
    if (b < bc) terms[b] = lp[(size_t)b * V + target[b]];
}
void launch_pppl_pick(const float* lp, const int32_t* target, int bc, int V, float* terms, hipStream_t s) {
    hipLaunchKernelGGL(pppl_pick_kernel, dim3((bc + 255) / 256), dim3(256), 0, s, lp, target, bc, V, terms);
}

// ... 330 lines not shown
```

### proteingym_amd/csrc/gemm16x_kernel.h

```cpp
#pragma once
#include <type_traits>

#include "common.h"

namespace pgmi {

typedef _Float16 h8 __attribute__((ext_vector_type(8)));
typedef _Float16 h4 __attribute__((ext_vector_type(4)));
typedef __bf16 b8 __attribute__((ext_vector_type(8)));
typedef unsigned int u32x4 __attribute__((ext_vector_type(4)));
typedef unsigned int u32x2 __attribute__((ext_vector_type(2)));

__device__ __forceinline__ f32x4 gelu_erf16(f32x4 x) {
    auto all = [](float v) { return f32x4{v, v, v, v}; };
    const f32x4 b = __builtin_elementwise_max(-__builtin_elementwise_abs(x), all(-6.0f));
    f32x4 q = __builtin_elementwise_fma(x, all(0.0f), all(3.309269596e-05f));
    q = __builtin_elementwise_fma(q, b, all(7.692188374e-04f));
    q = __builtin_elementwise_fma(q, b, all(8.080714382e-03f));
    q = __builtin_elementwise_fma(q, b, all(5.341210216e-02f));
    q = __builtin_elementwise_fma(q, b, all(-4.587709904e-01f));
    q = __builtin_elementwise_fma(q, b, all(1.151201725e+00f));
    q = __builtin_elementwise_fma(q, b, all(-9.999930859e-01f));
    const f32x4 e = {__builtin_amdgcn_exp2f(q[0]), __builtin_amdgcn_exp2f(q[1]), __builtin_amdgcn_exp2f(q[2]), __builtin_amdgcn_exp2f(q[3])};
    return __builtin_elementwise_fma(b, e, __builtin_elementwise_max(x, all(0.0f)));
// ... 210 lines not shown
#pragma unroll
            for (int p = 0; p < 2; ++p)
#pragma unroll
                for (int j = 0; j < TN; ++j)
#pragma unroll
                    for (int i = 0; i < TH; ++i) acc[j][H * TH + i] = mfma16x16<true>(wf[p][j], af[p][i], acc[j][H * TH + i]);
            return;
        }
        if constexpr (H == 0) scale_whi();
#pragma unroll
        for (int j = 0; j < TN; ++j)
#pragma unroll
            for (int i = 0; i < TH; ++i) acc[j][H * TH + i] = mfma16x16<false>(wf[1][j], af[0][i], acc[j][H * TH + i]);
#pragma unroll
        for (int j = 0; j < TN; ++j)
#pragma unroll
            for (int i = 0; i < TH; ++i) acc[j][H * TH + i] = mfma16x16<false>(whs[j], af[1][i], acc[j][H * TH + i]);
#pragma unroll
        for (int j = 0; j < TN; ++j)
#pragma unroll
            for (int i = 0; i < TH; ++i) acc[j][H * TH + i] = mfma16x16<false>(wf[0][j], af[0][i], acc[j][H * TH + i]);
        if constexpr (H == 0) {
#pragma unroll
            for (int k = 0; k < 4 * TN; ++k) {
                __builtin_amdgcn_sched_group_barrier(0x008, 1, 0);
                __builtin_amdgcn_sched_group_barrier(0x002, 1, 0);
            }
            __builtin_amdgcn_sched_group_barrier(0x008, 3 * TN * TH - 4 * TN, 0);
        }
    };
    using H0 = std::integral_constant<int, 0>;
    using H1 = std::integral_constant<int, 1>;

    int item = blockIdx.x;
    if (item >= n_items) return;
    decode(item);
    issue_tile(0, 0);
    auto run_item = [&](auto tmc) -> bool {
        constexpr int TM = decltype(tmc)::value;
        phase_vm();
#pragma unroll
        for (int j = 0; j < TN; ++j)
#pragma unroll
            for (int i = 0; i < TM; ++i)
#pragma unroll
                for (int v = 0; v < 4; ++v) acc[j][i][v] = 0.0f;
        int cur = 0;
        if (late) phase();
        for (int kt = 0; kt < nk; ++kt) {
            const u32x4* Ab = lds + cur * X_STAGE;
            const u32x4* Wb = Ab + X_OP_CH;
            __builtin_amdgcn_s_setprio(0);
            if (kt + 1 < nk) issue_tile(kt + 1, cur ^ 1);
            read_frags(tmc, H0{}, Ab, Wb);
            phase();
            __builtin_amdgcn_s_setprio(1);
            mfmas(tmc, H0{});
            phase();
            __builtin_amdgcn_s_setprio(0);
            read_frags(tmc, H1{}, Ab, Wb);
            if (late) phase_vm(); else phase();
            __builtin_amdgcn_s_setprio(1);
            mfmas(tmc, H1{});
            if (!late) phase_vm(); else phase();
            cur ^= 1;
        }
        __builtin_amdgcn_s_setprio(0);
        if (!late) phase();

        const int em0 = m0, en0 = n0, eb = batch;
        item += gridDim.x;
        const bool more = item < n_items;
        if (more) {
            decode(item);
            issue_tile(0, 0);
        }

        if constexpr (OUT == 2) {
            const int Dm = N / 3;
            const int nb = en0 + wn * 64;
            if (nb < N) {
            const int which = nb / Dm, hcol = nb - which * Dm, hh = hcol >> 6;
            constexpr int SPQ = 144;
            unsigned char* patch_q = patches + wave * (2 * 32 * SPQ);
            const bool staged_q = which < 2;
            f32x4 bq0[2], bq1[2];
#pragma unroll
            for (int g = 0; g < 2; ++g) {
                bq0[g] = *reinterpret_cast<const f32x4*>(bias + nb + 16 * g + 4 * kq);
                bq1[g] = *reinterpret_cast<const f32x4*>(bias + nb + 32 + 16 * g + 4 * kq);
            }
#pragma unroll
            for (int g = 0; g < 2; ++g) asm volatile("" :: "v"(bq0[g]), "v"(bq1[g]));
            auto emit = [&](auto interior_c) {
            constexpr bool INT = decltype(interior_c)::value;
            unsigned char* const lane_cell = patch_q + r * SPQ + kq * 8;
            unsigned short* const int_dst = !INT ? nullptr : Ch + (size_t)(em0 + wm * TM * 16 + (lane >> 3)) * (2 * Dm) + (size_t)which * Dm + hcol + (lane & 7) * 8;
#pragma unroll
            for (int ib = 0; ib < TM / 2; ++ib) {
#pragma unroll
            for (int s = 0; s < 2; ++s) {
                const int i = 2 * ib + s;
                const int m = em0 + (wm * TM + i) * 16 + r;
                const bool row_ok = m < M;
                if (!INT && !row_ok) continue;
                int bb = 0, t = 0;
                if (!INT || qo.rotary) {
                    bb = m / qo.T;
                    t = m - bb * qo.T;
                }
                f32x4 rc[2], rs[2];
                if ((INT || which < 2) && qo.rotary) {
                    const int tr = (min(t, qo.T - 1) * qo.rot_halves + (hh % qo.rot_halves)) * 64;
#pragma unroll
                    for (int g = 0; g < 2; ++g) {
                        rc[g] = *reinterpret_cast<const f32x4*>(qo.cos_t + tr + 16 * g + 4 * kq);
                        rs[g] = *reinterpret_cast<const f32x4*>(qo.sin_t + tr + 16 * g + 4 * kq);
                    }
                }
#pragma unroll
                for (int g = 0; g < 2; ++g) {
                    const int d0 = 16 * g + 4 * kq;
                    const f32x4 b0 = bq0[g], b1 = bq1[g];
                    float x0[4], x1[4];
#pragma unroll
                    for (int e = 0; e < 4; ++e) {
                        x0[e] = fmaf(acc[g][i][e], out_scale, b0[e]);
                        x1[e] = fmaf(acc[g + 2][i][e], out_scale, b1[e]);
                    }
                    if (which == 0) {
#pragma unroll
                        for (int e = 0; e < 4; ++e) { x0[e] *= kQLog2e; x1[e] *= kQLog2e; }
                    }
                    if (INT || which < 2) {
                        if (qo.rotary) {
                            const f32x4 c1 = rc[g], s1 = rs[g], c2 = rc[g], s2 = rs[g];
#pragma unroll
                            for (int e = 0; e < 4; ++e) {
                                const float y0 = fmaf(x0[e], c1[e], (-x1[e]) * s1[e]);
                                const float y1 = fmaf(x1[e], c2[e], x0[e] * s2[e]);
                                x0[e] = y0;
                                x1[e] = y1;
                            }
                        }
                        h4 hi0, lo0, hi1, lo1;
                        split_act4(f32x4{x0[0], x0[1], x0[2], x0[3]}, hi0, lo0);
                        split_act4(f32x4{x1[0], x1[1], x1[2], x1[3]}, hi1, lo1);
                        unsigned char* cell = lane_cell + (16 * s) * SPQ + 32 * g;
                        lds_put(cell, hi0);
                        lds_put(cell + 32 * SPQ, lo0);
                        lds_put(cell + 64, hi1);
                        lds_put(cell + 32 * SPQ + 64, lo1);
                    } else {
                        const int tk = t & 31;
                        const int pos = (t & ~31) + ((tk & 0x13) | ((tk & 4) << 1) | ((tk & 8) >> 1));
                        unsigned short* col = qo.vt16 + (((size_t)bb * qo.H + hh) * kHeadDim + d0) * qo.Tp + pos;
#pragma unroll
                        for (int e = 0; e < 4; ++e) {
                            _Float16 a0, l0, a1, l1;
                            split_act(x0[e], a0, l0);
                            split_act(x1[e], a1, l1);
                            unsigned short* c0 = col + (size_t)e * qo.Tp;
                            unsigned short* c1p = c0 + (size_t)32 * qo.Tp;
                            c0[0] = __builtin_bit_cast(unsigned short, a0);
                            c0[qo.vt_plane] = __builtin_bit_cast(unsigned short, l0);
                            c1p[0] = __builtin_bit_cast(unsigned short, a1);
                            c1p[qo.vt_plane] = __builtin_bit_cast(unsigned short, l1);
                        }
                    }
                }
            }
                if (INT || staged_q) {
                    __builtin_amdgcn_wave_barrier();
                    const int m_base = em0 + (wm * TM + 2 * ib) * 16;
#pragma unroll
                    for (int k = 0; k < 4; ++k) {
                        const int q = lane + 64 * k, row = q >> 3, cc = q & 7;
                        const u32x4 vh = *reinterpret_cast<const u32x4*>(patch_q + row * SPQ + cc * 16);
                        const u32x4 vl = *reinterpret_cast<const u32x4*>(patch_q + (32 + row) * SPQ + cc * 16);
                        if (INT || m_base + row < M) {
                            unsigned short* dst = INT ? int_dst + (size_t)(32 * ib + 8 * k) * (size_t)(2 * Dm)
                                                      : Ch + (size_t)(m_base + row) * (2 * Dm) + (size_t)which * Dm + hcol + cc * 8;
                            *reinterpret_cast<u32x4*>(dst) = vh;
                            *reinterpret_cast<u32x4*>(dst + c_plane) = vl;
                        }
                    }
                    __builtin_amdgcn_wave_barrier();
                }
            }
            };
            if (staged_q && em0 + (wm + 1) * (TM * 16) <= M) emit(std::true_type{});
            else emit(std::false_type{});
            }
        } else if constexpr (OUT == 0) {
            unsigned char* patch = patches + wave * (32 * 128);
            const int cc = lane & 7, rq = lane >> 3;
            const unsigned int kOob = 0x80000000u;
            const unsigned int ldc = xm.ldc ? (unsigned int)xm.ldc : (unsigned int)N;
            const long long cb = xm.tiles_per_batch ? (long long)(eb % xm.batch_inner) * xm.c_b0 + (long long)(eb / xm.batch_inner) * xm.c_b1 : 0;
            const __amdgpu_buffer_rsrc_t rsC = __builtin_amdgcn_make_buffer_rsrc(Cf + cb, 0, (int)((unsigned int)M * ldc * 4u), 0x00020000);
            const __amdgpu_buffer_rsrc_t rsR = __builtin_amdgcn_make_buffer_rsrc(const_cast<float*>(residual ? residual : Cf) + cb, 0, (int)((unsigned int)M * ldc * 4u), 0x00020000);
            constexpr int NB = TN / 2;
            unsigned int coff[NB];
            f32x4 bv[NB];
#pragma unroll
            for (int j = 0; j < NB; ++j) {
                const int n = en0 + wn * 64 + j * 32 + cc * 4;
                coff[j] = n < N ? (unsigned int)n * 4u : kOob;
                bv[j] = (bias && n < N) ? *reinterpret_cast<const f32x4*>(bias + n) : f32x4{0.f, 0.f, 0.f, 0.f};
            }
#pragma unroll
            for (int j = 0; j < NB; ++j) asm volatile("" :: "v"(bv[j]));
            auto c_off = [&](int m, int j) -> int {
                return (int)((m < M && coff[j] != kOob) ? (unsigned int)m * ldc * 4u + coff[j] : kOob);
            };
            u32x4 rv[2][NB][4];
            auto load_residual = [&](int i, u32x4 (&dst)[NB][4]) {
                const int m_base = em0 + (wm * TM + 2 * i) * 16;
#pragma unroll
                for (int j = 0; j < NB; ++j)
#pragma unroll
                    for (int k = 0; k < 4; ++k)
                        dst[j][k] = __builtin_bit_cast(u32x4, __builtin_amdgcn_raw_buffer_load_b128(rsR, c_off(m_base + rq + 8 * k, j), 0, 0));
            };
            if (residual) load_residual(0, rv[0]);
#pragma unroll
            for (int i = 0; i < TM / 2; ++i) {
                const int m_base = em0 + (wm * TM + 2 * i) * 16;
                if (residual && i + 1 < TM / 2) load_residual(i + 1, rv[(i + 1) & 1]);
#pragma unroll
                for (int j = 0; j < NB; ++j) {
#pragma unroll
                    for (int s = 0; s < 2; ++s)
#pragma unroll
                        for (int u = 0; u < 2; ++u) {
                            const int prow = 16 * s + r;
                            *reinterpret_cast<f32x4*>(patch + prow * 128 + (((4 * u + kq) ^ (prow & 7)) << 4)) = acc[2 * j + u][2 * i + s];
                        }
                    __builtin_amdgcn_wave_barrier();
#pragma unroll
                    for (int k = 0; k < 4; ++k) {
                        const int row = rq + 8 * k;
                        const f32x4 a = *reinterpret_cast<const f32x4*>(patch + row * 128 + ((cc ^ (row & 7)) << 4));
                        f32x4 val;
#pragma unroll
                        for (int e = 0; e < 4; ++e) val[e] = fmaf(a[e], out_scale, bv[j][e]);
                        if (EPI == EPI_GELU) val = gelu_erf16(val);
                        if (EPI == EPI_GELU_TANH) val = gelu_tanh16(val);
                        if (EPI == EPI_SQRELU)
#pragma unroll
                        for (int e = 0; e < 4; ++e) { const float t = fmaxf(val[e], 0.0f); val[e] = t * t; }
                        if (EPI == EPI_RELU)
#pragma unroll
                        for (int e = 0; e < 4; ++e) val[e] = fmaxf(val[e], 0.0f);
                        if (residual) {
                            const f32x4 rr = __builtin_bit_cast(f32x4, rv[i & 1][j][k]);
#pragma unroll
                            for (int e = 0; e < 4; ++e) val[e] = rr[e] + val[e];
                        }
                        __builtin_amdgcn_raw_buffer_store_b128(__builtin_bit_cast(u32x4, val), rsC, c_off(m_base + row, j), 0, 0);
                    }
                    __builtin_amdgcn_wave_barrier();
                }
            }
        } else {
            if constexpr (BF) {
                constexpr int SPB = 144;
                const bool staged = (N % 8 == 0) && (en0 + (wn + 1) * 64 <= N);
                unsigned char* patch = patches + wave * (32 * SPB);
                f32x4 bvs[TN];
#pragma unroll
                for (int j = 0; j < TN; ++j) {
                    const int n = en0 + wn * 64 + 16 * j + 4 * kq;
                    bvs[j] = (bias && n < N) ? *reinterpret_cast<const f32x4*>(bias + n) : f32x4{0.f, 0.f, 0.f, 0.f};
                }
#pragma unroll
                for (int j = 0; j < TN; ++j) asm volatile("" :: "v"(bvs[j]));
#pragma unroll
                for (int ib = 0; ib < TM / 2; ++ib) {
#pragma unroll
                    for (int s = 0; s < 2; ++s) {
                    const int i = 2 * ib + s, prow = 16 * s + r;
                    const int m = em0 + (wm * TM + i) * 16 + r;
                    if (m >= M) continue;
#pragma unroll
                    for (int j = 0; j < TN; ++j) {
                            const int n = en0 + wn * 64 + 16 * j + 4 * kq;
                            if (n >= N) continue;
                            const f32x4 bv = bvs[j];
                            f32x4 val;
#pragma unroll
                            for (int e = 0; e < 4; ++e) val[e] = fmaf(acc[j][i][e], out_scale, bv[e]);
                            if (EPI == EPI_GELU) val = gelu_erf16(val);
                            if (EPI == EPI_GELU_TANH) val = gelu_tanh16(val);
                            if (EPI == EPI_SQRELU)
#pragma unroll
                            for (int e = 0; e < 4; ++e) { const float t = fmaxf(val[e], 0.0f); val[e] = t * t; }
                            if (EPI == EPI_RELU)
#pragma unroll
                            for (int e = 0; e < 4; ++e) val[e] = fmaxf(val[e], 0.0f);
                            u32x2 pk;
                            pk[0] = (unsigned int)f32_to_bf16_rne(val[0]) | ((unsigned int)f32_to_bf16_rne(val[1]) << 16);
                            pk[1] = (unsigned int)f32_to_bf16_rne(val[2]) | ((unsigned int)f32_to_bf16_rne(val[3]) << 16);
                            if (staged) lds_put(patch + prow * SPB + (16 * j + 4 * kq) * 2, pk);
                            else *reinterpret_cast<u32x2*>(Ch + (size_t)m * (size_t)N + n) = pk;
                        }
                    }
                    if (staged) {
// ... 162 lines not shown
```

### proteingym_amd/csrc/model.h

```cpp
#pragma once
#include <math.h>
#include <stdlib.h>
#include <cmath>
#include <algorithm>
#include <stdarg.h>
#include <stdio.h>
#include <string.h>

#include <string>
#include <vector>

#include "common.h"
#include "gemm16x_kernel.h"
#include "packed_chunks.h"

namespace pgmi {

struct W16 {
    unsigned short* p = nullptr;
    float out_scale = 1.0f;
};

struct Layer {
    float *ln1_w, *ln1_b, *wqkv, *bqkv, *wo, *bo, *ln2_w, *ln2_b, *w1, *b1, *w2, *b2;
    W16 wqkv16, wo16, w116, w216;
    int ffn = 0;
    float* conv = nullptr;
    float *c_ln_w = nullptr, *c_ln_b = nullptr, *c_bqkv = nullptr, *c_bo = nullptr;
    W16 c_wqkv16, c_wo16;
    float* c_bq = nullptr;
    W16 c_wq16;
    float *q_ln = nullptr, *k_ln = nullptr;
    float* gate = nullptr;
    std::vector<W16> ew1, ew2;
    float *g_norm_w = nullptr, *g_wrot = nullptr, *g_wdist = nullptr;
    W16 g_proj16, g_out16;
};

struct ProfEvent {
    hipEvent_t start, stop;
    int cls;
};

struct PrefixCache {
    unsigned short* planes = nullptr;
    size_t pitch = 0, plane = 0, cap = 0;
    int rows = 0;
    int32_t* meta = nullptr;
    static size_t plan_ints(size_t cap) { return 3 * cap + 2; }
    static size_t meta_ints(size_t cap) { return 2 * plan_ints(cap) + cap + 4; }
    unsigned short* k(int l) const { return planes ? planes + (size_t)l * 4 * plane : nullptr; }
    unsigned short* vt(int l) const { return planes ? k(l) + 2 * plane : nullptr; }
    int32_t* plan(int slot) const { return meta + (size_t)slot * plan_ints(cap); }
    int32_t* seq_off() const { return plan(2); }
};

}

using namespace pgmi;

struct pgmi_assay;
struct pgmi_pppl;

struct pgmi_model {
    pgmi_config cfg;
    int device = 0;
    hipStream_t stream = nullptr;
    std::vector<void*> allocs;
    std::vector<pgmi_assay*> assays;
    std::vector<pgmi_pppl*> pppls;
    float *embed_tokens = nullptr, *embed_positions = nullptr;
    float *lnb_w = nullptr, *lnb_b = nullptr, *lna_w = nullptr, *lna_b = nullptr;
    float *hd_w = nullptr, *hd_b = nullptr, *hln_w = nullptr, *hln_b = nullptr;
    float *head_w = nullptr, *head_b = nullptr;
    std::vector<Layer> layers;
    W16 hd16;
    int fc1_epi = EPI_GELU, fc1_cols = 0;
    bool embed_gather = false;
    int mask_id = PGMI_TOK_MASK, n_token_ids = PGMI_VOCAB;
    float* slopes = nullptr;
    float* tr_prior = nullptr;
    size_t tr_prior_cap = 0;
    int32_t* tr_meta = nullptr;
    size_t tr_meta_cap = 0;
    int pg2_rotary = 0;
    float *pg2_aa_w = nullptr, *pg2_aa_b = nullptr;
    int gpt_Vp = 0, gpt_head_rows = 0;
    bool parallel_residual = false;
    float* gpt_logits = nullptr;
    W16 gpt_head16;
    double* gpt_sum = nullptr;
    bool rms_norm = false;
    int pg3_E = 0, pg3_k = 0, pg3_gated = 0;
    struct MoeWs {
        int32_t *ids = nullptr, *slot = nullptr, *blk_cnt = nullptr, *blk_base = nullptr, *counts_seg = nullptr;
        float *wts = nullptr, *y = nullptr, *t32 = nullptr;
        unsigned short *a16 = nullptr, *g16 = nullptr;
        int32_t* counts_host = nullptr;
        size_t layer_stride = 0;
    } moe;
    float* msa_pe = nullptr;
    float* xt = nullptr;
    int32_t *msa_full = nullptr, *msa_kv_len = nullptr;
    size_t msa_full_cap = 0;
    float *tied_part = nullptr, *tied_p = nullptr, *tied_vt = nullptr;
    size_t tied_part_cap = 0, tied_p_cap = 0, tied_vt_cap = 0;
    int msa_kv_R = 0, msa_kv_C = 0;
    float ln_eps = 1e-5f;
    bool final_norm = false;
    PrefixCache pfx;
    std::vector<float> poet_prompt_lp;
    int if1_enc = 0, if1_pos_len = 0;
    float *if1_mem = nullptr, *if1_pos = nullptr;
    unsigned short* if1_mem16 = nullptr;
    int e3_vheads = 0, e3_Kp = 0;
    float *e3_struct_embed = nullptr, *e3_const = nullptr;
    int32_t *e3_stok = nullptr, *e3_plddt = nullptr, *e3_mask = nullptr;
    float *e3_rot = nullptr, *e3_trans = nullptr;
    size_t e3_cap = 0;
    int e3_T = 0;
    bool e3_framed = false;
    int mu_groups = 0;
    float *mu_w = nullptr, *mu_b = nullptr, *mu_lna_w = nullptr, *mu_lna_b = nullptr;
    Layer mu_layer;
    float *mu_angles = nullptr, *mu_plddt = nullptr;
    size_t mu_angles_cap = 0, mu_plddt_cap = 0;
    int mu_T = 0;
    unsigned short *h16 = nullptr, *g16 = nullptr;
    size_t h16_plane = 0, g16_plane = 0;
    unsigned short *qk16 = nullptr, *vt16 = nullptr;
    size_t qk16_plane = 0, vt16_plane = 0;
    int32_t* nonfinite = nullptr;
    int gemm_variant = 0;
    int keep_rows = 1;
    int last_B = 0, last_T = 0;
    int dh = kHeadDim;
    int rot_halves = 1;
    int Hs = 0;
    int Da = 0;
    float *rot_cos = nullptr, *rot_sin = nullptr;
    int rot_len = 0;
    float* zeros = nullptr;
    int max_rows = 0;
    float *x = nullptr, *h = nullptr, *qkv = nullptr, *g = nullptr, *lp = nullptr, *denom = nullptr;
    int32_t *tokens = nullptr, *pos_idx = nullptr, *kv_len = nullptr, *row_idx = nullptr, *aux_i = nullptr;
    bool prof = false;
    std::vector<ProfEvent> events;
    size_t events_used = 0;
    double prof_ms[PGMI_K_COUNT] = {0};
    int64_t prof_n[PGMI_K_COUNT] = {0};
    double prof_flops[PGMI_K_COUNT] = {0};
    double prof_bytes[PGMI_K_COUNT] = {0};
};

struct pgmi_assay {
    pgmi_model* m = nullptr;
    int n_tok = 0, P = 0, T = 0;
    int64_t n_mut = 0, n_sub = 0;
    std::vector<void*> allocs;
    int32_t *wt = nullptr, *positions = nullptr, *win_start = nullptr, *mask_rel = nullptr;
    int32_t *sub_pos = nullptr, *sub_wt = nullptr, *sub_mt = nullptr;
    int64_t* mut_off = nullptr;
    float* table = nullptr;
    double* scores = nullptr;
};

struct pgmi_pppl {
    pgmi_model* m = nullptr;
    int64_t N = 0;
    std::vector<int64_t> off;
    std::vector<void*> allocs;
    uint8_t* tok8 = nullptr;
    int64_t* off_dev = nullptr;
    int64_t last_rows = 0, last_chunks = 0, last_tokens = 0, last_padded = 0;
};

namespace pgmi {

template <typename T>
int dev_alloc(std::vector<void*>& pool, T** p, size_t n) {
    void* q = nullptr;
    if (n == 0) n = 1;
    hipError_t e = hipMalloc(&q, n * sizeof(T));
    if (e != hipSuccess) {
        set_error("hipMalloc(%zu bytes) failed: %s", n * sizeof(T), hipGetErrorString(e));
        return PGMI_ENOMEM;
    }
    pool.push_back(q);
    *p = static_cast<T*>(q);
    return PGMI_OK;
}

template <typename T>
int dev_upload(std::vector<void*>& pool, T** p, const T* host, size_t n) {
    int rc = dev_alloc(pool, p, n);
    if (rc) return rc;
    if (n) PGMI_HIP(hipMemcpy(*p, host, n * sizeof(T), hipMemcpyHostToDevice));
    return PGMI_OK;
}

struct ProfScope {
    pgmi_model* m;
    bool on = false;
    size_t idx = 0;
    ProfScope(pgmi_model* m_, int cls, double flops, double bytes) : m(m_) {
        if (!m->prof) return;
        if (m->events_used == m->events.size()) {
            ProfEvent e;
            if (hipEventCreate(&e.start) != hipSuccess || hipEventCreate(&e.stop) != hipSuccess) return;
            m->events.push_back(e);
        }
        idx = m->events_used++;
        on = true;
        m->events[idx].cls = cls;
        m->prof_n[cls] += 1;
        m->prof_flops[cls] += flops;
        m->prof_bytes[cls] += bytes;
        hipEventRecord(m->events[idx].start, m->stream);
    }
    ProfScope(const ProfScope&) = delete;
    ~ProfScope() {
        if (on) hipEventRecord(m->events[idx].stop, m->stream);
    }
};

template <typename T>
int ensure_cap(pgmi_model* m, T** p, size_t* cap, size_t need) {
    if (need <= *cap) return PGMI_OK;
    T* q = nullptr;
    int rc = dev_alloc(m->allocs, &q, need);
    if (rc) return rc;
    *p = q;
    *cap = need;
    return PGMI_OK;
}

template <typename T>
constexpr T roundup32(T v) { return (v + 31) / 32 * 32; }

template <typename T>
struct DevBuf {
    T* p = nullptr;
    size_t cap = 0;
    int reserve(pgmi_model* m, size_t n) { return ensure_cap(m, &p, &cap, n); }
    operator T*() const { return p; }
};

inline int reserve_all(pgmi_model*) { return PGMI_OK; }
template <typename T, typename... Rest>
int reserve_all(pgmi_model* m, DevBuf<T>& b, size_t n, Rest&&... rest) {
    const int rc = b.reserve(m, n);
    return rc ? rc : reserve_all(m, rest...);
}

int prof_drain(pgmi_model* m);
int side_open(pgmi_model* pm, const char* name, const float* w, int64_t n_weights, int64_t want, bool scan_finite, int device, int precision,
              hipStream_t lend);
int side_sync(pgmi_model* pm, int rc, const char* what);
int overflow_error(int precision);
void side_release(pgmi_model* pm, bool own_stream);
int check_cfg(const pgmi_config* c);
int check_tokens(const int32_t* tokens, int B, int T, int n_ids = PGMI_VOCAB);
int check_vocab(const int32_t* tokens, int B, int T, int V);
int env_int(const char* name, int dflt);
int make_w16(std::vector<void*>& pool, const float* host, size_t n, size_t K, int precision, hipStream_t s, W16* out);
int linear(pgmi_model* m, const float* in32, const unsigned short* in16, const float* W32, const W16& w16, const float* bias,
           const float* residual, float* out32, unsigned short* out16, int M, int N, int K, int epi);
GemmLaunch qkv_launch(pgmi_model* m, const W16& w16, const float* bias, int M, int Da, int K, int T, int H);
PrefixAttLaunch prefix_launch(pgmi_model* m, const SegPlan& pl);
int alloc_prefix_cache(pgmi_model* m);
int check_nonfinite(pgmi_model* m);
int reset_pad_keys(pgmi_model* m, int B, int T);
int model_create(const pgmi_config* cfg, const float* w, int64_t n_weights, int device, pgmi_model** out, int arch_arg,
                 const pgmi_pg3_params* pg3 = nullptr);
struct BlobCursor;
void walk_esm(BlobCursor& c);
void walk_esm_layer(BlobCursor& c, Layer* L, size_t F);
int encoder_layer(pgmi_model* m, const Layer& L, int B, int T, bool rotary, const int32_t* keep = nullptr, int n_keep = 0,
                  bool* compacted = nullptr);
int create_esm(pgmi_model* m, const pgmi_config* cfg, const float* w, int64_t n_weights);
int ensure_rotary(pgmi_model* m, int T);
int upload_rotate_half(pgmi_model* m, int n);
int run_encoder(pgmi_model* m, int B, int T, const int32_t* keep = nullptr, int n_keep = 0, bool* compacted = nullptr);
int head_hidden(pgmi_model* m, int R, const int32_t* row_idx);
int run_head(pgmi_model* m, int R, const int32_t* row_idx);
int run_rows(pgmi_model* m, int B, int T, int R, const int32_t* row_idx);
int create_tranception(pgmi_model* m, const pgmi_config* cfg, const float* w, int64_t n_weights);
int create_progen2(pgmi_model* m, const pgmi_config* cfg, const float* w, int64_t n_weights, int rotary_dim);
int create_gpt(pgmi_model* m, const pgmi_config* cfg, const float* w, int64_t n_weights, int pos_kind);
int64_t gpt_weight_count(const pgmi_config* c, int pos_kind);
int decoder_check(pgmi_model* m, int arch, int T);
int run_decoder(pgmi_model* m, int B, int T, const AttRagged* rg = nullptr, int rows = 0, double att_flops = 0);
int self_attention(pgmi_model* m, const Layer& L, int B, int T, const AttRagged* rg = nullptr, int rows = 0, double att_flops = 0);
int out_proj(pgmi_model* m, const W16& wo16, const float* bo, int M);
int ffn(pgmi_model* m, const Layer& L, int M);
int narrow_head(pgmi_model* m, const float* src, int n);
int loglik_tail(pgmi_model* m, const int32_t* row_idx, int R, const int32_t* d_off, int bc, double* sum);
int decoder_token_logprobs(pgmi_model* m, int arch, const int32_t* tokens, int B, int T, float* out);
int decoder_sequence_loglik(pgmi_model* m, int arch, const int32_t* tokens, const int32_t* lens, int B, int T, double* sum, int32_t* n_targets);
int pg3_check(const pgmi_config* c, const pgmi_pg3_params* p);
int64_t pg3_weight_count(const pgmi_config* c, const pgmi_pg3_params* p);
int create_progen3(pgmi_model* m, const pgmi_config* cfg, const float* w, int64_t n_weights, const pgmi_pg3_params* p);
void pack_swiglu(const float* w1, const float* w3, size_t F, size_t D, float* dst);
int moe_ws_alloc(std::vector<void*>& pool, pgmi_model::MoeWs* ws, size_t rows, size_t layers, int D, int F, int E, int top_k, int gated);
int dense_ffn(pgmi_model* m, const pgmi_model::MoeWs& ws, const W16& w1, const W16& w2, const unsigned short* h16, unsigned short* g16,
              int M, int D, int F, int gated, float* x);
int pg3_ffn(pgmi_model* m, const Layer& L, int layer, int M);
int moe_ffn(pgmi_model* m, const pgmi_model::MoeWs& ws, const std::vector<W16>& ew1, const std::vector<W16>& ew2,
            const unsigned short* h16, const int32_t* ids, const float* wts, int M, int D, int F, int E, int top_k, int gated, float* x);
int64_t poet_weight_count(const pgmi_config* c, int final_norm);
int create_poet(pgmi_model* m, const pgmi_config* cfg, const float* w, int64_t n_weights, int final_norm);
struct PackedScorer {
    int (*forward)(pgmi_model* m, int bc, int R, const SegPlan& pl);
    int pos_len;
    const char* pos_what;
    const char* not_ready;
    bool same_length;
    bool vocab_per_row;
    int skip_target;
    bool mean;
};
int score_packed(pgmi_model* m, const PackedScorer& e, const int32_t* tokens, const int32_t* lens, int B, int T, bool loglik, float* out,
                 double* sum);
int if1_check(const pgmi_config* c, int enc_dim);
int64_t if1_weight_count(const pgmi_config* c, int enc_dim);
int create_esmif1(pgmi_model* m, const pgmi_config* cfg, const float* w, int64_t n_weights, int enc_dim);
int64_t esmc_weight_count(const pgmi_config* c);
int create_esmc(pgmi_model* m, const pgmi_config* cfg, const float* w, int64_t n_weights);
int esm3_check(const pgmi_config* c, int v_heads);
int64_t esm3_weight_count(const pgmi_config* c, int v_heads);
int create_esm3(pgmi_model* m, const pgmi_config* cfg, const float* w, int64_t n_weights, int v_heads);
int esm3_embed(pgmi_model* m, int B, int T);
int geom_branch(pgmi_model* m, const Layer& L, int B, int T);
int create_saprot(pgmi_model* m, const pgmi_config* cfg, const float* w, int64_t n_weights, int mask_id);
int64_t mulan_weight_count(const pgmi_config* c);
int create_mulan(pgmi_model* m, const pgmi_config* cfg, const float* w, int64_t n_weights, int mask_id);
int mulan_embed(pgmi_model* m, int B, int T);
int create_msa(pgmi_model* m, const pgmi_config* cfg, const float* w, int64_t n_weights);
int run_msa(pgmi_model* m, int R, int C, int keep_col = -1, bool* compacted = nullptr);

inline bool esm2_rotary(int arch) { return arch == PGMI_ARCH_ESM2 || arch == PGMI_ARCH_SAPROT || arch == PGMI_ARCH_MULAN; }
inline bool esmc_blocks(int arch) { return arch == PGMI_ARCH_ESMC || arch == PGMI_ARCH_ESM3; }

struct BlobCursor {
    pgmi_model* m;
    const float *p, *end;
    int rc = PGMI_OK;
    BlobCursor(pgmi_model* m_, const float* w, int64_t n_weights) : m(m_), p(w), end(w + n_weights) {}
    const float* take(size_t n) { p += n; return p - n; }
    void upload(float** dst, const float* host, size_t n) { if (!rc) rc = dev_upload(m->allocs, dst, host, n); }
    void upload(float** dst, size_t n) { upload(dst, take(n), n); }
    void upload(float** dst, const std::vector<float>& host) { upload(dst, host.data(), host.size()); }
    void w16(W16* dst, const float* host, size_t n, size_t K) { if (!rc) rc = make_w16(m->allocs, host, n, K, m->cfg.precision, m->stream, dst); }
    void w16(W16* dst, size_t n, size_t K) { w16(dst, take(n), n, K); }
    void linear(float** w32, W16* w16_, const float* host, size_t n, size_t K) {
        if (m->cfg.precision == PGMI_PREC_FP32) upload(w32, host, n); else w16(w16_, host, n, K);
    }
    void linear(float** w32, W16* w16_, size_t n, size_t K) { linear(w32, w16_, take(n), n, K); }
    void linear(float** w32, W16* w16_, const std::vector<float>& host, size_t K) { linear(w32, w16_, host.data(), host.size(), K); }
    int finish() {
        if (!rc && p != end) { set_error("internal: blob walk mismatch"); rc = PGMI_EINVAL; }
        return rc;
    }
};

inline float rebuild_split(unsigned short h, unsigned short l) {
    _Float16 a, b;
    memcpy(&a, &h, 2); memcpy(&b, &l, 2);
    return (float)a + (float)b * (1.0f / kLoScale);
}

struct OpScope {
    const char* what;
    int rc = PGMI_OK;
    pgmi_model tmp{};
    std::vector<void*>& pool = tmp.allocs;
    hipEvent_t ev[2] = {nullptr, nullptr};
    bool opened = false;

    OpScope(const char* what_, int device) : what(what_) {
        rc = open(device);
        opened = rc == PGMI_OK;
        if (rc == PGMI_EHIP) (void)hipGetLastError();
    }
    OpScope(const OpScope&) = delete;
    ~OpScope() {
        for (hipEvent_t e : ev)
            if (e) hipEventDestroy(e);
        if (tmp.moe.counts_host) hipHostFree(tmp.moe.counts_host);
        for (void* p : pool) hipFree(p);
    }
    int hip(hipError_t e) {
        if (!rc && e != hipSuccess) { set_error("%s failed: %s", what, hipGetErrorString(e)); rc = PGMI_EHIP; }
        return rc;
    }
    template <typename T>
    T* alloc(size_t n, int fill = -1) {
        T* p = nullptr;
        if (!rc) rc = dev_alloc(pool, &p, n);
        if (!rc && fill >= 0) hip(hipMemset(p, fill, n * sizeof(T)));
        return rc ? nullptr : p;
    }
    template <typename T>
    T* up(const T* host, size_t n) {
        T* p = nullptr;
        if (!rc) rc = dev_upload(pool, &p, host, n);
        return rc ? nullptr : p;
    }
    template <typename T>
    T* up(const std::vector<T>& host) { return up(host.data(), host.size()); }
    W16 w16(const float* host, size_t n, size_t K, int precision = PGMI_PREC_F16X3) {
        W16 w;
        if (!rc) rc = make_w16(pool, host, n, K, precision, nullptr, &w);
        return w;
    }
    int sync() {
        if (!opened) return rc;
        hipError_t e = hipDeviceSynchronize();
        if (e == hipSuccess) e = hipGetLastError();
        return hip(e);
    }
    template <typename T>
    void down(T* host, const T* dev, size_t n) {
        if (!rc) hip(hipMemcpy(host, dev, n * sizeof(T), hipMemcpyDeviceToHost));
    }
    void planes(float* host, const unsigned short* dev16, size_t rows, size_t cols) {
        std::vector<unsigned short> h(rc ? 0 : rows * cols * 2);
        down(h.data(), dev16, h.size());
        for (size_t r = 0; r < rows && !rc; ++r)
            for (size_t c = 0; c < cols; ++c) {
                const size_t o = ki_off(r, (int)c, (int)cols);
                host[r * cols + c] = rebuild_split(h[o], h[o + 32]);
            }
    }
    void bf16_plane(float* host, const unsigned short* dev16, size_t n) {
        std::vector<unsigned short> h(rc ? 0 : n);
        down(h.data(), dev16, n);
        for (size_t i = 0; i < n && !rc; ++i) {
            const unsigned int u = (unsigned int)h[i] << 16;
// ... 95 lines not shown
```

Baseline: 18110.

## Share layer-0 QKV across masked windows and run kept-row attention by tile

Masked windows with the same start differ only at the masked position. Layer 0 LayerNorm and the QKV GEMM therefore run on a deduplicated set of a wild-type plus a masked sequence per window group, and the per-row Q/K and V^T planes are rebuilt with a gather/patch copy kernel. In the last layer, attention is computed only for the 32-query tile holding each kept row instead of all queries. The vocab log-softmax kernel is also restructured to spread vocab dot products across 16 waves per row. This adds host-side share planning, extra copy kernels and scratch reuse of the qkv buffer, and exactness depends on layer 0 being position-local apart from attention.

```diff
diff --git a/proteingym_amd/csrc/api_esm.hip b/proteingym_amd/csrc/api_esm.hip
--- a/proteingym_amd/csrc/api_esm.hip
+++ b/proteingym_amd/csrc/api_esm.hip
@@ -69,7 +69,36 @@
     });
 }
 
-int encoder_layer(pgmi_model* m, const Layer& L, int B, int T, bool rotary, const int32_t* keep, int n_keep, bool* compacted) {
+static struct { int on = 1; bool set = false; } g_share;
+void share_options_from_env() {
+    if (!g_share.set) g_share.on = env_int("PGMI_SHARE_LAYER0", 1);
+}
+int share_set_option(const char* name, long long value) {
+    if (strcmp(name, "share_layer0")) return PGMI_EINVAL;
+    g_share.set = value >= 0;
+    if (value >= 0) g_share.on = (int)value; else share_options_from_env();
+    return PGMI_OK;
+}
+
+struct ShareScratch {
+    float* x = nullptr;
+    unsigned short *qk = nullptr, *vt = nullptr;
+    size_t qk_plane = 0, vt_plane = 0, bytes = 0;
+};
+static ShareScratch share_scratch(const pgmi_model* m, int n_seq, int T) {
+    const size_t rows = (size_t)n_seq * T, D = m->cfg.embed_dim, Da = m->Da;
+    ShareScratch sc;
+    sc.x = m->qkv;
+    sc.qk = reinterpret_cast<unsigned short*>(m->qkv + rows * D);
+    sc.qk_plane = rows * 2 * Da;
+    sc.vt = sc.qk + 2 * sc.qk_plane;
+    sc.vt_plane = (size_t)n_seq * Da * roundup32((size_t)T);
+    sc.bytes = rows * D * 4 + (2 * sc.qk_plane + 2 * sc.vt_plane) * 2;
+    return sc;
+}
+
+int encoder_layer(pgmi_model* m, const Layer& L, int B, int T, bool rotary, const int32_t* keep, int n_keep, bool* compacted,
+                  const SharedRows* share, const AttRagged* kept_tiles) {
     const pgmi_config& c = m->cfg;
     const int M = B * T, D = c.embed_dim, F = L.ffn ? L.ffn : c.ffn_dim, N1 = L.ffn ? L.ffn : m->fc1_cols, H = c.heads, Da = m->Da;
     hipStream_t s = m->stream;
@@ -77,20 +106,35 @@
     const double ln_bytes = 2.0 * M * D * 4;
     const int prec = c.precision;
     const int mode16 = (prec == PGMI_PREC_F16X3) ? 1 : 2;
-    { ProfScope p(m, PGMI_K_LAYERNORM, 0, ln_bytes);
+    const int Ms = share ? share->n_seq * T : M;
+    const ShareScratch sc = share ? share_scratch(m, share->n_seq, T) : ShareScratch{};
+    { ProfScope p(m, PGMI_K_LAYERNORM, 0, share ? 3.0 * Ms * D * 4 : ln_bytes);
+      if (share) launch_gather_rows(m->x, share->gather, Ms, D, sc.x, s);
       if (prec == PGMI_PREC_FP32) launch_layernorm(m->x, L.ln1_w, L.ln1_b, M, D, 1e-5f, m->h, s);
-      else launch_layernorm16(m->x, L.ln1_w, L.ln1_b, M, D, 1e-5f, m->h16, mode16, s); }
+      else launch_layernorm16(share ? sc.x : m->x, L.ln1_w, L.ln1_b, Ms, D, 1e-5f, m->h16, mode16, s); }
     const bool fused_qkv = prec != PGMI_PREC_FP32 && !L.q_ln;
-    { ProfScope p(m, PGMI_K_GEMM_QKV, 2.0 * M * 3 * D * D, 0);
+    { ProfScope p(m, PGMI_K_GEMM_QKV, 2.0 * Ms * 3 * D * D, share ? 2.0 * M * 3 * Da * 4 : 0);
       if (fused_qkv) {
-          GemmLaunch g = qkv_launch(m, L.wqkv16, L.bqkv, M, Da, D, T, m->Hs);
+          GemmLaunch g = qkv_launch(m, L.wqkv16, L.bqkv, Ms, Da, D, T, m->Hs);
           g.bf = prec == PGMI_PREC_BF16;
           g.qkv.cos_t = m->rot_cos; g.qkv.sin_t = m->rot_sin; g.qkv.rotary = rotary; g.qkv.rot_halves = m->rot_halves;
+          if (share) {
+              g.out16 = sc.qk; g.qkv.qk_plane = sc.qk_plane;
+              g.qkv.vt16 = sc.vt; g.qkv.vt_plane = sc.vt_plane;
+          }
           rc = launch_gemm16(g);
+          if (share && !rc) {
+              ShareCopy cp;
+              cp.s_qk = sc.qk; cp.s_qk_plane = sc.qk_plane; cp.s_vt = sc.vt; cp.s_vt_plane = sc.vt_plane;
+              cp.seq_wt = share->seq_wt; cp.seq_mask = share->seq_mask; cp.mask_rel = share->mask_rel;
+              cp.B = B; cp.T = T; cp.Da = Da;
+              cp.qk16 = m->qk16; cp.qk_plane = m->qk16_plane; cp.vt16 = m->vt16; cp.vt_plane = m->vt16_plane;
+              launch_share_copy(cp, s);
+          }
       } else
           rc = linear(m, m->h, m->h16, L.wqkv, L.wqkv16, L.bqkv, nullptr, m->qkv, nullptr, M, 3 * Da, D, EPI_NONE);
       if (rc) return rc; }
-    { ProfScope p(m, PGMI_K_ATTENTION, 4.0 * M * T * D, L.q_ln ? (double)M * D * 20 : 0);
+    { ProfScope p(m, PGMI_K_ATTENTION, 4.0 * (kept_tiles ? 32 * kept_tiles->n_blocks : M) * T * D, L.q_ln ? (double)M * D * 20 : 0);
       if (L.q_ln && (rc = launch_qkln_prep(m->qkv, L.q_ln, L.k_ln, 1e-5f, m->rot_cos, m->rot_sin, B, T, H, m->qk16, m->qk16_plane,
                                            m->vt16, m->vt16_plane, s)))
           return rc;
@@ -104,7 +148,7 @@
           a.out = prec == PGMI_PREC_F16X3 ? ATT_OUT_SPLIT : ATT_OUT_BF16;
           a.ctx16 = m->h16;
           a.stream = s;
-          rc = launch_attention_f16x3_v2(a);
+          rc = kept_tiles ? launch_attention_kept_tiles(a, *kept_tiles) : launch_attention_f16x3_v2(a);
       } else {
           rc = launch_attention_f32(m->qkv, m->kv_len, B, T, H, m->h, s, m->rot_halves * kHeadDim);
       }
@@ -148,7 +192,7 @@
     return PGMI_OK;
 }
 
-int run_encoder(pgmi_model* m, int B, int T, const int32_t* keep, int n_keep, bool* compacted) {
+int run_encoder(pgmi_model* m, int B, int T, const int32_t* keep, int n_keep, bool* compacted, const SharedRows* share) {
     const pgmi_config& c = m->cfg;
     const int M = B * T, D = c.embed_dim;
     hipStream_t s = m->stream;
@@ -171,9 +215,19 @@
             launch_zero_pad_rows(m->tokens, M, D, m->x, s);
         }
     }
+    const Layer& L0 = m->layers[0];
+    const Layer& Ll = m->layers[c.layers - 1];
+    const bool plain = c.arch != PGMI_ARCH_MULAN && c.arch != PGMI_ARCH_SAPROT && c.arch != PGMI_ARCH_ESM3 && !L0.q_ln && !L0.g_norm_w &&
+                       !Ll.q_ln && !Ll.g_norm_w;
+    const bool shared = share && share->n_seq > 0 && m->keep_rows && g_share.on && c.precision != PGMI_PREC_FP32 && plain &&
+                        2 * share->n_seq < B && share_scratch(m, share->n_seq, T).bytes <= (size_t)m->max_rows * 3 * m->Da * 4;
     for (int l = 0; l < c.layers; ++l) {
         const bool kept = keep && m->keep_rows && l == c.layers - 1;
-        if ((rc = encoder_layer(m, m->layers[l], B, T, esm2_rotary(c.arch), kept ? keep : nullptr, n_keep, compacted))) return rc;
+        const bool tiles = kept && share && share->kept.n_blocks == B && n_keep == B && c.precision != PGMI_PREC_FP32 && plain &&
+                           m->rot_halves == 1;
+        if ((rc = encoder_layer(m, m->layers[l], B, T, esm2_rotary(c.arch), kept ? keep : nullptr, n_keep, compacted,
+                                l == 0 && shared ? share : nullptr, tiles ? &share->kept : nullptr)))
+            return rc;
     }
     PGMI_HIP(hipGetLastError());
     return PGMI_OK;
@@ -208,11 +262,71 @@
 }
 
 
-int run_rows(pgmi_model* m, int B, int T, int R, const int32_t* row_idx) {
+int run_rows(pgmi_model* m, int B, int T, int R, const int32_t* row_idx, const SharedRows* share) {
     bool compacted = false;
-    int rc = run_encoder(m, B, T, row_idx, R, &compacted);
+    int rc = run_encoder(m, B, T, row_idx, R, &compacted, share);
     if (rc) return rc;
     return run_head(m, R, compacted ? nullptr : row_idx);
+}
+
+static int build_share(pgmi_assay* a, int p0, int bc, SharedRows* out) {
+    const int T = a->T;
+    const int32_t *ws = a->win_start_h.data() + p0, *mr = a->mask_rel_h.data() + p0;
+    std::vector<int32_t> gather, seq_wt(bc), seq_mask(bc);
+    int n_seq = 0;
+    for (int c0 = 0, c1; c0 < bc; c0 = c1) {
+        for (c1 = c0 + 1; c1 < bc && ws[c1] == ws[c0];) ++c1;
+        const bool pair = c1 - c0 >= 3;
+        const int s0 = n_seq;
+        n_seq += pair ? 2 : c1 - c0;
+        gather.resize((size_t)n_seq * T);
+        if (!pair) {
+            for (int b = c0; b < c1; ++b) {
+                seq_wt[b] = seq_mask[b] = s0 + (b - c0);
+                for (int t = 0; t < T; ++t) gather[(size_t)seq_wt[b] * T + t] = b * T + t;
+            }
+            continue;
+        }
+        int32_t *gw = &gather[(size_t)s0 * T], *gm = gw + T;
+        for (int t = 0; t < T; ++t) {
+            int b = c0;
+            while (b < c1 && mr[b] == t) ++b;
+            if (b == c1) b = c0;
+            gw[t] = gm[t] = b * T + t;
+        }
+        for (int b = c0; b < c1; ++b) {
+            gm[mr[b]] = b * T + mr[b];
+            seq_wt[b] = s0;
+            seq_mask[b] = s0 + 1;
+        }
+    }
+    out->mask_rel = a->mask_rel + p0;
+    const size_t vt_blk = (size_t)a->m->Da * roundup32((size_t)T);
+    std::vector<int32_t> row0(bc), zero(bc, 0), seq(bc), tile(bc);
+    std::vector<uint32_t> vt(bc);
+    for (int b = 0; b < bc; ++b) {
+        row0[b] = b * T; seq[b] = b; tile[b] = mr[b] / 32;
+        vt[b] = (uint32_t)(b * vt_blk);
+    }
+    int32_t *d_row0 = nullptr, *d_zero = nullptr, *d_seq = nullptr, *d_tile = nullptr;
+    uint32_t* d_vt = nullptr;
+    int rc = dev_upload(a->allocs, &d_row0, row0.data(), row0.size());
+    if (!rc) rc = dev_upload(a->allocs, &d_zero, zero.data(), zero.size());
+    if (!rc) rc = dev_upload(a->allocs, &d_seq, seq.data(), seq.size());
+    if (!rc) rc = dev_upload(a->allocs, &d_tile, tile.data(), tile.size());
+    if (!rc) rc = dev_upload(a->allocs, &d_vt, vt.data(), vt.size());
+    if (rc) return rc;
+    out->kept.seq_off = d_row0; out->kept.seq_p = d_zero; out->kept.seq_q = d_row0; out->kept.seq_root = d_seq; out->kept.seq_vt = d_vt;
+    out->kept.blk_seq = d_seq; out->kept.blk_j = d_tile; out->kept.n_blocks = bc;
+    if (2 * n_seq >= bc) return PGMI_OK;
+    int32_t *d_gather = nullptr, *d_wt = nullptr, *d_mask = nullptr;
+    rc = dev_upload(a->allocs, &d_gather, gather.data(), gather.size());
+    if (!rc) rc = dev_upload(a->allocs, &d_wt, seq_wt.data(), seq_wt.size());
+    if (!rc) rc = dev_upload(a->allocs, &d_mask, seq_mask.data(), seq_mask.size());
+    if (rc) return rc;
+    out->n_seq = n_seq;
+    out->gather = d_gather; out->seq_wt = d_wt; out->seq_mask = d_mask;
+    return PGMI_OK;
 }
 
 }
@@ -307,6 +421,12 @@
     if (!rc) rc = dev_upload(a->allocs, &a->mut_off, mut_off, (size_t)(n_mut + 1));
     if (!rc) rc = dev_alloc(a->allocs, &a->table, (size_t)n_tok * PGMI_VOCAB);
     if (!rc) rc = dev_alloc(a->allocs, &a->scores, (size_t)n_mut);
+    a->win_start_h = ws;
+    a->mask_rel_h = mr;
+    const bool wt_masked = std::find(wt_tokens, wt_tokens + n_tok, m->mask_id) != wt_tokens + n_tok;
+    const int per = rows_per_chunk(m, T);
+    a->share.resize(wt_masked ? 0 : (P + per - 1) / per);
+    for (size_t i = 0; i < a->share.size() && !rc; ++i) rc = build_share(a, (int)i * per, std::min(per, P - (int)i * per), &a->share[i]);
     if (rc) { pgmi_assay_destroy(a); return rc; }
     m->assays.push_back(a);
     *out = a;
@@ -336,7 +456,8 @@
         const int bc = std::min(per, a->P - p0);
         launch_make_masked_windows(a->wt, a->win_start + p0, a->mask_rel + p0, bc, T, m->tokens, s);
         launch_row_index(a->mask_rel + p0, bc, T, m->row_idx, s);
-        int rc = run_rows(m, bc, T, bc, m->row_idx);
+        const size_t chunk = (size_t)(p0 / per);
+        int rc = run_rows(m, bc, T, bc, m->row_idx, chunk < a->share.size() ? &a->share[chunk] : nullptr);
         if (rc) return rc;
         launch_scatter_rows(m->lp, a->positions + p0, bc, V, a->table, s);
     }
diff --git a/proteingym_amd/csrc/api_model.hip b/proteingym_amd/csrc/api_model.hip
--- a/proteingym_amd/csrc/api_model.hip
+++ b/proteingym_amd/csrc/api_model.hip
@@ -416,6 +416,7 @@
     if (rc) { pgmi_model_destroy(m); return rc; }
     m->keep_rows = env_int("PGMI_KEEP_ROWS", 1);
     gemm_options_from_env();
+    share_options_from_env();
     m->gemm_variant = env_int("PGMI_GEMM_VARIANT", 0);
     *out = m;
     return PGMI_OK;
@@ -505,7 +506,8 @@
     if (rc) rc = mpnn_set_option(name, (long long)value);
     if (rc) rc = unirep_set_option(name, (long long)value);
     if (rc) rc = s2f_set_option(name, (long long)value);
-    if (rc) set_error("unknown option '%s' (gemm_half_tail, gemm_max_rows, att_xcd_local, att_v3, eve_max_rows, eve_fixed_sample, eve_prior_batch, mpnn_max_rows, unirep_max_rows, s2f_max_rows)", name);
+    if (rc) rc = share_set_option(name, (long long)value);
+    if (rc) set_error("unknown option '%s' (gemm_half_tail, gemm_max_rows, share_layer0, att_xcd_local, att_v3, eve_max_rows, eve_fixed_sample, eve_prior_batch, mpnn_max_rows, unirep_max_rows, s2f_max_rows)", name);
     return rc;
 }
 
diff --git a/proteingym_amd/csrc/attention_f16.hip b/proteingym_amd/csrc/attention_f16.hip
--- a/proteingym_amd/csrc/attention_f16.hip
+++ b/proteingym_amd/csrc/attention_f16.hip
@@ -284,6 +284,7 @@
     att16v2_inst<1, ATT_OUT_SPLIT, 3, 64>(), att16v2_inst<2, ATT_OUT_SPLIT, 3, 64>(), att16v2_inst<4, ATT_OUT_SPLIT, 3, 64>(),
     att16v2_inst<1, ATT_OUT_BF16, 3, 64>(),  att16v2_inst<2, ATT_OUT_BF16, 3, 64>(),  att16v2_inst<4, ATT_OUT_BF16, 3, 64>(),
     att16v2_inst<1, ATT_OUT_SPLIT, 3, 64, true>(), att16v2_inst<2, ATT_OUT_SPLIT, 3, 64, true>(), att16v2_inst<4, ATT_OUT_SPLIT, 3, 64, true>(),
+    att16v2_inst<1, ATT_OUT_BF16, 3, 64, true>(),
     att16v2_inst<4, ATT_OUT_F32, 3, 128>(),  att16v2_inst<4, ATT_OUT_SPLIT, 3, 128>(), att16v2_inst<4, ATT_OUT_BF16, 3, 128>(),
     att16v2_inst<4, ATT_OUT_SPLIT, 2, 256, false, 128>(),
 };
@@ -380,4 +381,16 @@
     return launch_att16v2(a, att16_waves_per_block(T), dim3(rg.n_blocks, H, 1), &rag, 0);
 }
 
-}
+int launch_attention_kept_tiles(const AttLaunch& a, const AttRagged& rg) {
+    if (a.T <= 0 || a.H <= 0 || a.qkv || a.conv || a.slopes || a.head_dim != 64 || (a.out != ATT_OUT_SPLIT && a.out != ATT_OUT_BF16) ||
+        rg.n_blocks <= 0) {
+        set_error("attention_kept_tiles: bad arguments T=%d H=%d out=%d head_dim=%d entries=%d", a.T, a.H, (int)a.out, a.head_dim, rg.n_blocks);
+        return PGMI_EINVAL;
+    }
+    const int rc = check_operand_range("attention_kept_tiles", a);
+    if (rc) return rc;
+    const RagMap rag{rg.seq_off, rg.seq_p, rg.seq_q, rg.seq_root, rg.seq_vt, rg.blk_seq, rg.blk_j};
+    return launch_att16v2(a, 1, dim3(rg.n_blocks, a.H, 1), &rag, 0);
+}
+
+}
diff --git a/proteingym_amd/csrc/common.h b/proteingym_amd/csrc/common.h
--- a/proteingym_amd/csrc/common.h
+++ b/proteingym_amd/csrc/common.h
@@ -34,6 +34,10 @@
 
 __host__ __device__ __forceinline__ size_t ki_off(size_t row, int k, int K) {
     return row * (size_t)(2 * K) + (size_t)(k >> 5) * 64 + (size_t)(k & 31);
+}
+__host__ __device__ __forceinline__ int vt_key_slot(int t) {
+    const int tk = t & 31;
+    return (t & ~31) + ((tk & 0x13) | ((tk & 4) << 1) | ((tk & 8) >> 1));
 }
 #if defined(__HIPCC__)
 __device__ __forceinline__ void split_act(float x, _Float16& hi, _Float16& lo) {
@@ -94,6 +98,17 @@
 void launch_layernorm(const float* x, const float* w, const float* b, int rows, int D, float eps,
                       float* y, hipStream_t s);
 void launch_gather_rows(const float* x, const int32_t* row_idx, int n, int D, float* y, hipStream_t s);
+struct ShareCopy {
+    const unsigned short* s_qk = nullptr;
+    const unsigned short* s_vt = nullptr;
+    size_t s_qk_plane = 0, s_vt_plane = 0;
+    const int32_t *seq_wt = nullptr, *seq_mask = nullptr, *mask_rel = nullptr;
+    int B = 0, T = 0, Da = 0;
+    unsigned short* qk16 = nullptr;
+    unsigned short* vt16 = nullptr;
+    size_t qk_plane = 0, vt_plane = 0;
+};
+void launch_share_copy(const ShareCopy& c, hipStream_t s);
 void launch_strided_index(int first, int stride, int n, int32_t* idx, hipStream_t s);
 void launch_vocab_logsoftmax(const float* h, const float* E, const float* bias, int rows, int D,
                              int V, float* out, int32_t* nonfinite, hipStream_t s);
@@ -421,5 +436,6 @@
 int att16_waves_per_block(int T);
 int att_set_option(const char* name, long long value);
 int launch_attention_tr_ragged(const AttLaunch& a, const AttRagged& rg);
-
-}
+int launch_attention_kept_tiles(const AttLaunch& a, const AttRagged& rg);
+
+}
diff --git a/proteingym_amd/csrc/elementwise.hip b/proteingym_amd/csrc/elementwise.hip
--- a/proteingym_amd/csrc/elementwise.hip
+++ b/proteingym_amd/csrc/elementwise.hip
@@ -307,6 +307,51 @@
     hipLaunchKernelGGL(gather_rows_kernel, dim3((n + 3) / 4), dim3(256), 0, s, x, idx, n, D, y);
 }
 
+typedef unsigned int share_u32x4 __attribute__((ext_vector_type(4)));
+__global__ __launch_bounds__(256) void share_qk_kernel(ShareCopy c) {
+    const int row = blockIdx.x * 4 + (threadIdx.x >> 6);
+    const int lane = threadIdx.x & 63;
+    if (row >= c.B * c.T) return;
+    const int b = row / c.T, t = row - b * c.T;
+    const int seq = (t == c.mask_rel[b]) ? c.seq_mask[b] : c.seq_wt[b];
+    const int n16 = c.Da / 4;
+    const unsigned short* src = c.s_qk + ((size_t)seq * c.T + t) * (size_t)(2 * c.Da);
+    unsigned short* dst = c.qk16 + (size_t)row * (size_t)(2 * c.Da);
+    for (int i = lane; i < n16; i += 64) {
+        reinterpret_cast<share_u32x4*>(dst)[i] = reinterpret_cast<const share_u32x4*>(src)[i];
+        reinterpret_cast<share_u32x4*>(dst + c.qk_plane)[i] = reinterpret_cast<const share_u32x4*>(src + c.s_qk_plane)[i];
+    }
+}
+__global__ __launch_bounds__(256) void share_vt_kernel(ShareCopy c, int Tp) {
+    const int tp8 = Tp / 8, n = c.Da * tp8;
+    const int ch = blockIdx.x * 256 + threadIdx.x;
+    if (ch >= n) return;
+    const int b = blockIdx.y;
+    const int col0 = (ch % tp8) * 8;
+    const int mr = c.mask_rel[b], mcol = vt_key_slot(mr) - col0;
+    const size_t blk = (size_t)c.Da * Tp, off = (size_t)ch * 8;
+    const unsigned short* w = c.s_vt + (size_t)blockIdx.z * c.s_vt_plane + (size_t)c.seq_wt[b] * blk + off;
+    const unsigned short* k = c.s_vt + (size_t)blockIdx.z * c.s_vt_plane + (size_t)c.seq_mask[b] * blk + off;
+    unsigned short* d = c.vt16 + (size_t)blockIdx.z * c.vt_plane + (size_t)b * blk + off;
+    if ((col0 & ~31) + 32 <= c.T) {
+        union { share_u32x4 v; unsigned short h[8]; } u;
+        u.v = *reinterpret_cast<const share_u32x4*>(w);
+        const unsigned short kv = (mcol >= 0 && mcol < 8) ? k[mcol] : (unsigned short)0;
+#pragma unroll
+        for (int j = 0; j < 8; ++j)
+            if (j == mcol) u.h[j] = kv;
+        *reinterpret_cast<share_u32x4*>(d) = u.v;
+    } else {
+        for (int j = 0; j < 8; ++j)
+            if (vt_key_slot(col0 + j) < c.T) d[j] = (j == mcol) ? k[j] : w[j];
+    }
+}
+void launch_share_copy(const ShareCopy& c, hipStream_t s) {
+    const int Tp = (c.T + 31) / 32 * 32;
+    hipLaunchKernelGGL(share_qk_kernel, dim3((c.B * c.T + 3) / 4), dim3(256), 0, s, c);
+    hipLaunchKernelGGL(share_vt_kernel, dim3((c.Da * (Tp / 8) + 255) / 256, c.B, 2), dim3(256), 0, s, c, Tp);
+}
+
 __global__ void esm3_embed_kernel(const int32_t* __restrict__ tokens, const int32_t* __restrict__ stok, const int32_t* __restrict__ plddt,
                                   const float* __restrict__ seq_embed, const float* __restrict__ struct_embed, const float* __restrict__ cst,
                                   int n, int T, int D, float* __restrict__ x) {
@@ -360,23 +405,26 @@
     hipLaunchKernelGGL(fill_f32_kernel, dim3((unsigned)((n + 255) / 256)), dim3(256), 0, s, p, n, v);
 }
 
-__global__ __launch_bounds__(256) void vocab_logsoftmax_kernel(const float* __restrict__ h,
+constexpr int kVocabWaves = 16;
+__global__ __launch_bounds__(kVocabWaves * 64) void vocab_logsoftmax_kernel(const float* __restrict__ h,
                                                                const float* __restrict__ E,
                                                                const float* __restrict__ bias, int rows,
                                                                int D, int V, float* __restrict__ out,
                                                                int32_t* __restrict__ nonfinite) {
-    const int row = blockIdx.x * 4 + (threadIdx.x >> 6);
-    const int lane = threadIdx.x & 63;
-    if (row >= rows) return;
+    __shared__ double logits[kWave];
+    const int row = blockIdx.x;
+    const int lane = threadIdx.x & 63, wave = threadIdx.x >> 6;
     const float* hr = h + (size_t)row * D;
-    double my_logit = -INFINITY;
-    for (int v = 0; v < V; ++v) {
+    for (int v = wave; v < min(V, kWave); v += kVocabWaves) {
         const float* ev = E + (size_t)v * D;
         double acc = 0.0;
         for (int i = lane; i < D; i += 64) acc = fma((double)hr[i], (double)ev[i], acc);
         acc = wave_sum_d(acc);
-        if (lane == v) my_logit = acc + (double)bias[v];
-    }
+        if (lane == 0) logits[v] = acc + (double)bias[v];
+    }
+    __syncthreads();
+    if (wave != 0) return;
+    const double my_logit = (lane < V) ? logits[lane] : -INFINITY;
     const float mx = wave_max((float)my_logit);
     const double ex = (lane < V) ? exp(my_logit - (double)mx) : 0.0;
     const double lse = log(wave_sum_d(ex));
@@ -388,7 +436,7 @@
 }
 void launch_vocab_logsoftmax(const float* h, const float* E, const float* bias, int rows, int D, int V,
                              float* out, int32_t* nonfinite, hipStream_t s) {
-    hipLaunchKernelGGL(vocab_logsoftmax_kernel, dim3((rows + 3) / 4), dim3(256), 0, s, h, E, bias, rows, D, V, out, nonfinite);
+    hipLaunchKernelGGL(vocab_logsoftmax_kernel, dim3(rows), dim3(kVocabWaves * 64), 0, s, h, E, bias, rows, D, V, out, nonfinite);
 }
 
 __device__ __forceinline__ float fuse_eve(float two, float e, float beta, int eve_fallback) {
diff --git a/proteingym_amd/csrc/gemm16x_kernel.h b/proteingym_amd/csrc/gemm16x_kernel.h
--- a/proteingym_amd/csrc/gemm16x_kernel.h
+++ b/proteingym_amd/csrc/gemm16x_kernel.h
@@ -386,8 +386,7 @@
                         lds_put(cell + 64, hi1);
                         lds_put(cell + 32 * SPQ + 64, lo1);
                     } else {
-                        const int tk = t & 31;
-                        const int pos = (t & ~31) + ((tk & 0x13) | ((tk & 4) << 1) | ((tk & 8) >> 1));
+                        const int pos = vt_key_slot(t);
                         unsigned short* col = qo.vt16 + (((size_t)bb * qo.H + hh) * kHeadDim + d0) * qo.Tp + pos;
 #pragma unroll
                         for (int e = 0; e < 4; ++e) {
diff --git a/proteingym_amd/csrc/model.h b/proteingym_amd/csrc/model.h
--- a/proteingym_amd/csrc/model.h
+++ b/proteingym_amd/csrc/model.h
@@ -153,6 +153,12 @@
     double prof_bytes[PGMI_K_COUNT] = {0};
 };
 
+struct SharedRows {
+    int n_seq = 0;
+    const int32_t *gather = nullptr, *seq_wt = nullptr, *seq_mask = nullptr, *mask_rel = nullptr;
+    AttRagged kept{};
+};
+
 struct pgmi_assay {
     pgmi_model* m = nullptr;
     int n_tok = 0, P = 0, T = 0;
@@ -163,6 +169,8 @@
     int64_t* mut_off = nullptr;
     float* table = nullptr;
     double* scores = nullptr;
+    std::vector<int32_t> win_start_h, mask_rel_h;
+    std::vector<SharedRows> share;
 };
 
 struct pgmi_pppl {
@@ -277,14 +285,17 @@
 void walk_esm(BlobCursor& c);
 void walk_esm_layer(BlobCursor& c, Layer* L, size_t F);
 int encoder_layer(pgmi_model* m, const Layer& L, int B, int T, bool rotary, const int32_t* keep = nullptr, int n_keep = 0,
-                  bool* compacted = nullptr);
+                  bool* compacted = nullptr, const SharedRows* share = nullptr, const AttRagged* kept_tiles = nullptr);
+void share_options_from_env();
+int share_set_option(const char* name, long long value);
 int create_esm(pgmi_model* m, const pgmi_config* cfg, const float* w, int64_t n_weights);
 int ensure_rotary(pgmi_model* m, int T);
 int upload_rotate_half(pgmi_model* m, int n);
-int run_encoder(pgmi_model* m, int B, int T, const int32_t* keep = nullptr, int n_keep = 0, bool* compacted = nullptr);
+int run_encoder(pgmi_model* m, int B, int T, const int32_t* keep = nullptr, int n_keep = 0, bool* compacted = nullptr,
+                const SharedRows* share = nullptr);
 int head_hidden(pgmi_model* m, int R, const int32_t* row_idx);
 int run_head(pgmi_model* m, int R, const int32_t* row_idx);
-int run_rows(pgmi_model* m, int B, int T, int R, const int32_t* row_idx);
+int run_rows(pgmi_model* m, int B, int T, int R, const int32_t* row_idx, const SharedRows* share = nullptr);
 int create_tranception(pgmi_model* m, const pgmi_config* cfg, const float* w, int64_t n_weights);
 int create_progen2(pgmi_model* m, const pgmi_config* cfg, const float* w, int64_t n_weights, int rotary_dim);
 int create_gpt(pgmi_model* m, const pgmi_config* cfg, const float* w, int64_t n_weights, int pos_kind);
```

Result: no change. 18260, median of 6 (+0.8%).
